# chrisquince/DESMAN

Measured on AMD Instinct MI355X. Metric: Gibbs iterations/sec (VxS updates/s) at V=10k S=64 G=8, higher is better.
Workload: dtype f64; 1 GPU; synthetic V=10000 x S=64, G=8, full Gibbs iteration, 1 chain per GPU (configs[2]); V=10000, S=64, G=8, chains=1, tau_rng=mt19937

## Files before the change

### desman_amd/_lib.py

```python
import ctypes as C
import os

import numpy as np

_HERE = os.path.dirname(os.path.abspath(__file__))
LIB_PATH = os.environ.get("DESMAN_HIP_LIB") or os.path.join(_HERE, "lib", "libdesman_hip.so")
AB_LIB_PATH = os.path.join(_HERE, "lib", "libdesman_hip_ab.so")
HEADER_PATH = os.path.join(os.path.dirname(_HERE), "include", "desman_hip.h")

DSM_OK = 0
RNG_MT19937, RNG_PHILOX = 0, 1
STATS_AGG = 2
K_NAMES = ("stats", "dirichlet", "tau", "finalize", "mt", "nmft_a", "nmft_gamma", "nmft_b", "stats2", "stats_big", "stats_pat")


class DesmanHipError(RuntimeError):
    pass


_i64p = np.ctypeslib.ndpointer(np.int64, flags="C_CONTIGUOUS")
_f64p = np.ctypeslib.ndpointer(np.float64, flags="C_CONTIGUOUS")
_u64p = np.ctypeslib.ndpointer(np.uint64, flags="C_CONTIGUOUS")
_u32p = np.ctypeslib.ndpointer(np.uint32, flags="C_CONTIGUOUS")
_i32p = np.ctypeslib.ndpointer(np.int32, flags="C_CONTIGUOUS")
_vp, _i, _d = C.c_void_p, C.c_int, C.c_double

SIGNATURES = {
    "dsm_last_error": (C.c_char_p, []),
    "dsm_device_count": (_i, []),
    "dsm_version": (C.c_char_p, []),
    "dsm_initRNG": (_i, []),
    "dsm_setRNG": (_i, [C.c_ulong]),
    "dsm_freeRNG": (_i, []),
    "dsm_sample_tau": (_i, [_i64p, _f64p, _f64p, _i64p, _i, _i, _i]),
    "c_initRNG": (None, []),
    "c_setRNG": (None, [C.c_ulong]),
    "c_freeRNG": (None, []),
    "c_sample_tau": (_i, [_i64p, _f64p, _f64p, _i64p, _i, _i, _i]),
    "dsm_getRNG_state": (_i, [_u32p]),
    "dsm_setRNG_state": (_i, [_u32p]),
    "dsm_ctx_create": (_i, [C.POINTER(_vp), _i]),
    "dsm_ctx_destroy": (_i, [_vp]),
    "dsm_ctx_sync": (_i, [_vp]),
    "dsm_ctx_set_counts": (_i, [_vp, _i64p, _i, _i]),
    "dsm_ctx_set_state": (_i, [_vp, _i64p, _f64p, _f64p, _i]),
    "dsm_ctx_get_state": (_i, [_vp, _vp, _vp, _vp]),
    "dsm_ctx_set_gamma_eta": (_i, [_vp, _vp, _vp]),
    "dsm_ctx_set_priors": (_i, [_vp, _d, _d, _d]),
    "dsm_ctx_seed": (_i, [_vp, C.c_ulong, C.c_uint64]),
    "dsm_ctx_set_tau_rng": (_i, [_vp, _i]),
    "dsm_ctx_get_mt_state": (_i, [_vp, _u32p]),
    "dsm_ctx_set_mt_state": (_i, [_vp, _u32p]),
    "dsm_mt_seed_state": (_i, [C.c_ulong, _u32p]),
    "dsm_ctx_debug_mt_fill": (_i, [_vp, C.c_size_t, _u32p]),
    "dsm_ctx_sample_tau": (_i, [_vp, C.POINTER(_i), _vp]),
    "dsm_ctx_sample_stats": (_i, [_vp, C.c_uint32, _u64p, _u64p]),
    "dsm_ctx_stats_spec": (_i, [_vp]),
    "dsm_ctx_sweep_stats": (_i, [_vp, C.POINTER(C.c_uint64), C.POINTER(C.c_uint64), _i]),
    "dsm_ctx_set_tau_screen": (_i, [_vp, _i]),
    "dsm_ctx_set_tau_neartie": (_i, [_vp, _i]),
    "dsm_ctx_set_nmft_fused": (_i, [_vp, _i]),
    "dsm_ctx_set_nmft_persist": (_i, [_vp, _i]),
    "dsm_ctx_tau_launch_info": (_i, [_vp, C.POINTER(_i), C.POINTER(_i)]),
    "dsm_ctx_debug_log2f": (_i, [_vp, _vp, _vp, C.c_size_t]),
    "dsm_debug_fdiv": (_i, [_i, _f64p, _f64p, _f64p, _i]),
    "dsm_release_device_caches": (_i, []),
    "dsm_ctx_force_stats_spec": (_i, [_vp, _i]),
    "dsm_ctx_debug_stage1": (_i, [_vp, C.c_uint32, _vp, _u64p]),
    "dsm_ctx_debug_binom": (_i, [_vp, _i, C.c_uint32, _f64p, C.c_uint64, _i, _u32p, _i]),
    "dsm_ctx_draw_gamma_eta": (_i, [_vp, C.c_uint32, _u64p, _u64p, _f64p, _f64p]),
    "dsm_ctx_loglik": (_i, [_vp, C.POINTER(_d), C.POINTER(_d)]),
    "dsm_ctx_gibbs_update": (_i, [_vp, _i]),
    "dsm_ctx_get_counters": (_i, [_vp, C.POINTER(C.c_uint64), C.POINTER(C.c_uint32)]),
    "dsm_ctx_set_counters": (_i, [_vp, C.c_uint64, C.c_uint32]),
    "dsm_ctx_get_screen_state": (_i, [_vp, _u32p]),
    "dsm_ctx_set_screen_state": (_i, [_vp, _u32p]),
    "dsm_ctx_gibbs_update_sharded": (_i, [_vp, _i, _i, _i, _vp, _vp]),
    "dsm_ctx_gibbs_update_sharded_comm": (_i, [_vp, _i, _i, _i, _vp]),
    "dsm_comm_unique_id": (_i, [_vp]),
    "dsm_comm_create": (_i, [C.POINTER(_vp), _vp, _i, _i, _i]),
    "dsm_comm_destroy": (_i, [_vp]),
    "dsm_comm_rank": (_i, [_vp]),
    "dsm_comm_world": (_i, [_vp]),
    "dsm_comm_allgather_f64": (_i, [_vp, _f64p, _f64p, C.c_size_t]),
    "dsm_comm_allreduce_f64": (_i, [_vp, _vp, C.c_size_t, _i]),
    "dsm_comm_barrier": (_i, [_vp]),
    "dsm_device_read": (_i, [_i, _vp, _vp, C.c_size_t]),
    "dsm_device_write": (_i, [_i, _vp, _vp, C.c_size_t]),
    "dsm_batch_gibbs_update": (_i, [C.POINTER(_vp), _i, _i]),
    "dsm_batch_update_tau": (_i, [C.POINTER(_vp), _i, _i, C.POINTER(_vp), C.POINTER(_vp)]),
    "dsm_batch_nmft_factorize": (_i, [C.POINTER(_vp), _i, _i, _d, _i, C.POINTER(_i), _vp]),
    "dsm_ctx_update_tau": (_i, [_vp, _i, _f64p, _f64p]),
    "dsm_ctx_get_trace": (_i, [_vp, _vp, _vp, _vp, _vp, _vp]),
    "dsm_ctx_get_star": (_i, [_vp, _vp, _vp, _vp, C.POINTER(_d), C.POINTER(_i)]),
    "dsm_ctx_get_tau_sum": (_i, [_vp, _i64p]),
    "dsm_ctx_get_tau_at": (_i, [_vp, _i, _i64p]),
    "dsm_nmft_set": (_i, [_vp, _f64p, _f64p, _i]),
    "dsm_nmft_get": (_i, [_vp, _vp, _vp]),
    "dsm_nmft_factorize": (_i, [_vp, _i, _d, _i, C.POINTER(_i), _vp]),
    "dsm_nmft_objective": (_i, [_vp, C.POINTER(_d)]),
    "dsm_nmft_get_tau": (_i, [_vp, _i64p]),
    "dsm_lrt_step": (_i, [_i, _f64p, _i32p, _i32p, _f64p, _d, _i, _i, _f64p, _f64p, _f64p]),
    "dsm_assign_tau": (_i, [_i, _i64p, _i, _i, _i, _f64p, _f64p, C.c_uint64, _vp, _vp, _vp, _vp, _vp]),
    "dsm_ctx_assign_tau": (_i, [_vp, _f64p, _f64p, _i, C.c_uint64, _vp, _vp, _vp, _vp, _vp]),
    "dsm_assign_debug_set_chunk": (_i, [_i]),
    "dsm_genes_create": (_i, [C.POINTER(_vp), _i]),
    "dsm_genes_destroy": (_i, [_vp]),
    "dsm_genes_set_data": (_i, [_vp, _vp, _i, _i, _i, _i32p, _f64p]),
    "dsm_genes_set_model": (_i, [_vp, _f64p, _f64p, _f64p, _i, _i, _f64p, _f64p, _f64p]),
    "dsm_genes_set_state": (_i, [_vp, _vp, _vp]),
    "dsm_genes_get_state": (_i, [_vp, _vp, _vp]),
    "dsm_genes_seed": (_i, [_vp, C.c_ulong, C.c_uint64]),
    "dsm_genes_set_gene_base": (_i, [_vp, _i]),
    "dsm_genes_get_mt_state": (_i, [_vp, _u32p]),
    "dsm_genes_set_mt_state": (_i, [_vp, _u32p]),
    "dsm_genes_nmft_tau": (_i, [_vp, _vp, _f64p, _i, _d, _vp]),
    "dsm_genes_sweep_all": (_i, [_vp, _vp, _i, _vp, _vp, _vp]),
    "dsm_genes_step_candidates": (_i, [_vp, _i, _i, _f64p, _vp]),
    "dsm_genes_step_choose": (_i, [_vp, _i, _i, _i]),
    "dsm_genes_update": (_i, [_vp, _i, _i, _vp, _vp, _vp, _vp]),
    "dsm_genes_loglik": (_i, [_vp, _vp]),
    "dsm_genes_get_star": (_i, [_vp, _vp, _vp]),
    "dsm_genes_set_star": (_i, [_vp, _vp, _vp]),
    "dsm_kl_assign": (_i, [_i, _f64p, _f64p, _f64p, _i, _i, _i, _i, _d, C.POINTER(_i), C.POINTER(_d)]),
    "dsm_ctx_set_timing": (_i, [_vp, _i]),
    "dsm_ctx_get_timing": (_i, [_vp, _vp, _vp]),
    "dsm_kernel_name": (C.c_char_p, [_i]),
}

EXCHANGE_FN = C.CFUNCTYPE(C.c_int, C.c_void_p, C.c_void_p, C.c_size_t, C.c_void_p, C.c_size_t)
_lib = None


def _digest(a):
    try:
        import xxhash
        return xxhash.xxh3_128_digest(memoryview(a).cast("B"))
    except ImportError:
        import hashlib
        return hashlib.blake2b(memoryview(a).cast("B"), digest_size=16).digest()


def load():
    global _lib
    if _lib is None:
        if not os.path.exists(LIB_PATH):
            raise DesmanHipError(
                "libdesman_hip.so not built (%s); run `python -c 'import __graft_entry__ as g; g.build()'` "
                "or `make -C desman_amd/csrc`.  There is no CPU fallback." % LIB_PATH)
        try:
            lib = C.CDLL(LIB_PATH)
# ... 181 lines not shown
    def restore(self, ck):
        self.set_state(np.ascontiguousarray(ck["tau"], dtype=np.int64), np.ascontiguousarray(ck["gamma"], dtype=np.float64),
                       np.ascontiguousarray(ck["eta"], dtype=np.float64))
        mt = np.asarray(ck["mt_state"], dtype=np.uint32)
        if mt.size == 625:
            self.set_mt_state(np.ascontiguousarray(mt))
        check(self.lib.dsm_ctx_set_counters(self._h, int(ck["ctr_seed"]), int(ck["iter_ctr"])))
        self.set_screen_state(ck["screen"] if "screen" in ck else np.zeros(2, dtype=np.uint32))

    def set_mt_state(self, st):
        check(self.lib.dsm_ctx_set_mt_state(self._h, np.ascontiguousarray(st, dtype=np.uint32)))

    def debug_mt_fill(self, n):
        out = np.empty(int(n), dtype=np.uint32)
        check(self.lib.dsm_ctx_debug_mt_fill(self._h, int(n), out))
        return out

    def set_tau_rng(self, mode):
        check(self.lib.dsm_ctx_set_tau_rng(self._h, int(mode)))

    def assign_tau(self, gamma, eta, seed=None):
        gamma, eta = _assign_model(gamma, eta, self.S)
        G = gamma.shape[1]
        out = _assign_out(self.V, G, seed)
        check(self.lib.dsm_ctx_assign_tau(self._h, gamma, eta, G, int(seed or 0) & 0xFFFFFFFFFFFFFFFF, _ptr(out["map_state"]),
                                          _ptr(out["conf"]), _ptr(out["logz"]), _ptr(out["marg"]), _ptr(out.get("draw_state"))))
        return out

    def sample_tau(self, want_logp=False):
        n = _i(0)
        logp = np.empty((self.V, self.G, 4)) if want_logp else None
        check(self.lib.dsm_ctx_sample_tau(self._h, C.byref(n), _ptr(logp)))
        return (n.value, logp) if want_logp else n.value

    def sample_stats(self, it):
        mu = np.zeros((self.S, self.G), dtype=np.uint64)
        E = np.zeros((4, 4), dtype=np.uint64)
        check(self.lib.dsm_ctx_sample_stats(self._h, int(it), mu, E))
        return mu, E

    def debug_log2f(self, x):
        x = np.ascontiguousarray(x, dtype=np.float32)
        out = np.empty_like(x)
        check(self.lib.dsm_ctx_debug_log2f(self._h, x.ctypes.data, out.ctypes.data, x.size))
        return out

    def set_tau_neartie(self, mode=-1):
        check(self.lib.dsm_ctx_set_tau_neartie(self._h, int(mode)))

    def set_tau_screen(self, on):
        check(self.lib.dsm_ctx_set_tau_screen(self._h, 1 if on else 0))

    def tau_launch_info(self):
        a, b = _i(0), _i(0)
        check(self.lib.dsm_ctx_tau_launch_info(self._h, C.byref(a), C.byref(b)))
        return a.value, b.value

    def set_nmft_persist(self, mode=-1):
        check(self.lib.dsm_ctx_set_nmft_persist(self._h, int(mode)))

    def set_nmft_fused(self, mode=-1):
        check(self.lib.dsm_ctx_set_nmft_fused(self._h, int(mode)))

    def sweep_stats(self, reset=False):
        a, b = C.c_uint64(0), C.c_uint64(0)
        check(self.lib.dsm_ctx_sweep_stats(self._h, C.byref(a), C.byref(b), 1 if reset else 0))
        return a.value, b.value

    def stats_spec(self):
        r = self.lib.dsm_ctx_stats_spec(self._h)
        if r < 0:
            check(r)
        return r

    def force_stats_spec(self, spec=0):
        check(self.lib.dsm_ctx_force_stats_spec(self._h, int(spec)))

    def debug_stage1(self, it):
        nt = np.zeros((self.S, 1 << self.G), dtype=np.uint32)
        E = np.zeros((4, 4), dtype=np.uint64)
        check(self.lib.dsm_ctx_debug_stage1(self._h, int(it), nt.ctypes.data, E))
        return nt, E

    def debug_binom(self, kind, n, w, seed, nsamp, spec=STATS_AGG):
        w4 = np.zeros(4)
        w4[:len(w)] = w
        out = np.zeros((nsamp, 4) if kind == 2 else nsamp, dtype=np.uint32)
        check(self.lib.dsm_ctx_debug_binom(self._h, int(kind), int(n), w4, int(seed), int(nsamp), out.reshape(-1), int(spec)))
        return out

    def draw_gamma_eta(self, it, sum_mu, esum):
        g = np.empty((self.S, self.G)); e = np.empty((4, 4))
        check(self.lib.dsm_ctx_draw_gamma_eta(self._h, int(it), np.ascontiguousarray(sum_mu, dtype=np.uint64),
                                              np.ascontiguousarray(esum, dtype=np.uint64), g, e))
        return g, e

    def loglik(self):
        ll, lp = _d(0), _d(0)
        check(self.lib.dsm_ctx_loglik(self._h, C.byref(ll), C.byref(lp)))
        return ll.value, lp.value

    def gibbs_update(self, n_iter):
        check(self.lib.dsm_ctx_gibbs_update(self._h, int(n_iter)))
        self.n_trace = int(n_iter)

    def gibbs_update_sharded(self, n_iter, v_offset, v_total, exchange):
        err = []

        def cb(user, tab, n_tab, vec, n_vec):
            try:
                exchange(tab or 0, int(n_tab), vec, int(n_vec))
                return 0
            except BaseException as e:
                err.append(e)
                return 1
        fn = EXCHANGE_FN(cb)
        rc = self.lib.dsm_ctx_gibbs_update_sharded(self._h, int(n_iter), int(v_offset), int(v_total), C.cast(fn, _vp), None)
        if err:
            raise err[0]
        check(rc)
        self.n_trace = int(n_iter)

    def gibbs_update_sharded_comm(self, n_iter, v_offset, v_total, comm):
        check(self.lib.dsm_ctx_gibbs_update_sharded_comm(self._h, int(n_iter), int(v_offset), int(v_total), comm._h))
        self.n_trace = int(n_iter)

    @staticmethod
    def batch_gibbs_update(ctxs, n_iter):
        ctxs = list(ctxs)
        arr = (_vp * len(ctxs))(*[c._h.value for c in ctxs])
        check(load().dsm_batch_gibbs_update(arr, len(ctxs), int(n_iter)))
        for c in ctxs:
            c.n_trace = int(n_iter)

    def update_tau(self, gamma_store, eta_store):
        g = np.ascontiguousarray(gamma_store, dtype=np.float64)
        e = np.ascontiguousarray(eta_store, dtype=np.float64)
        check(self.lib.dsm_ctx_update_tau(self._h, g.shape[0], g, e))
        self.n_trace = g.shape[0]

    def get_trace(self):
        n = self.n_trace
        ll = np.empty(n); lp = np.empty(n); nch = np.empty(n, dtype=np.int32)
        g = np.empty((n, self.S, self.G)); e = np.empty((n, 4, 4))
        check(self.lib.dsm_ctx_get_trace(self._h, _ptr(ll), _ptr(lp), _ptr(nch), _ptr(g), _ptr(e)))
        return dict(ll=ll, lp=lp, nchange=nch, gamma=g, eta=e)

    def get_star(self):
        tau = np.empty((self.V, self.G, 4), dtype=np.int64)
        g = np.empty((self.S, self.G)); e = np.empty((4, 4))
        lp, it = _d(0), _i(0)
        check(self.lib.dsm_ctx_get_star(self._h, _ptr(tau), _ptr(g), _ptr(e), C.byref(lp), C.byref(it)))
        return dict(tau=tau, gamma=g, eta=e, lp=lp.value, it=it.value)

    def get_tau_sum(self):
        out = np.empty((self.V, self.G, 4), dtype=np.int64)
        check(self.lib.dsm_ctx_get_tau_sum(self._h, out))
        return out

    def get_tau_at(self, it):
        out = np.empty((self.V, self.G, 4), dtype=np.int64)
        check(self.lib.dsm_ctx_get_tau_at(self._h, int(it), out))
        return out

    def nmft_set(self, tau, gamma):
        tau = np.ascontiguousarray(tau, dtype=np.float64)
# ... 186 lines not shown
```

### desman_amd/csrc/api.hip

```cpp
#include <math.h>
#include <stdarg.h>
#include <stdio.h>
#include <string.h>

#include <algorithm>
#include <mutex>
#include <numeric>
#include <thread>

#include "dsm_host.h"
#include "log_table.h"

static thread_local char g_err[512] = "";

void dsm_set_error(const char *fmt, ...)
{
    va_list ap;
    va_start(ap, fmt);
    vsnprintf(g_err, sizeof g_err, fmt, ap);
    va_end(ap);
}

extern "C" const char *dsm_last_error(void) { return g_err; }
extern "C" const char *dsm_version(void) { return "desman_hip 0.1 (gfx950)"; }
// ... 113 lines not shown
    static const std::vector<uint32_t> ident = [] { std::vector<uint32_t> v((size_t)2 * DSM_MAX_GRID); for (size_t i = 0; i < v.size(); ++i) v[i] = (uint32_t)(i % DSM_MAX_GRID); return v; }();
    c->blk_order_n[0] = c->blk_order_n[1] = 0;
    if (!c->blk_order) return DSM_OK;
    HIP_TRY(hipMemcpyAsync(c->blk_order, ident.data(), ident.size() * sizeof(uint32_t), hipMemcpyHostToDevice, c->stream));
    return DSM_OK;
}

extern "C" int dsm_ctx_create(dsm_ctx **out, int device)
{
    if (!out) return DSM_ERR_ARG;
    *out = nullptr;
    int n = dsm_device_count();
    if (n <= 0) { dsm_set_error("no HIP device visible"); return DSM_ERR_NODEVICE; }
    if (device < 0 || device >= n) { dsm_set_error("device %d out of range (0..%d)", device, n - 1); return DSM_ERR_ARG; }
    HIP_TRY(hipSetDevice(device));
    hipDeviceProp_t prop;
    HIP_TRY(hipGetDeviceProperties(&prop, device));
    if (strncmp(prop.gcnArchName, "gfx950", 6) != 0) {
        dsm_set_error("device %d is %s; this library is built for gfx950 only", device, prop.gcnArchName);
        return DSM_ERR_NODEVICE;
    }
    dsm_ctx *c = new dsm_ctx();
    c->device = device;
    HIP_TRY(hipStreamCreateWithFlags(&c->stream, hipStreamNonBlocking));
    if (getenv("DESMAN_HIP_ONE_STREAM")) c->stream_rng = c->stream;
    else {
        int lo = 0, hi = 0;
        HIP_TRY(hipDeviceGetStreamPriorityRange(&lo, &hi));
        HIP_TRY(hipStreamCreateWithPriority(&c->stream_rng, hipStreamNonBlocking, hi));
    }
    for (int i = 0; i < 2; ++i) {
        HIP_TRY(hipEventCreateWithFlags(&c->ev_u_ready[i], hipEventDisableTiming));
        HIP_TRY(hipEventCreateWithFlags(&c->ev_u_free[i], hipEventDisableTiming));
    }
    TRY(dev_alloc(&c->mt_state, 625));
    TRY(dev_alloc(&c->ll_partial, 2 * DSM_MAX_GRID));
    TRY(dev_alloc(&c->nchange, 2));
    TRY(dev_alloc(&c->sweep_stats, 2));
    HIP_TRY(hipMemsetAsync(c->sweep_stats, 0, 2 * sizeof(unsigned long long), c->stream));
    TRY(dev_alloc(&c->step_cnt, (size_t)2 * 2 * DSM_MAX_GRID));
    HIP_TRY(hipMemsetAsync(c->step_cnt, 0, (size_t)2 * 2 * DSM_MAX_GRID * sizeof(uint32_t), c->stream));
    TRY(dev_alloc(&c->blk_order, (size_t)2 * DSM_MAX_GRID));
    TRY(reset_blk_order(c));
    TRY(dev_alloc(&c->screen_ctl, 4));
    HIP_TRY(hipMemsetAsync(c->screen_ctl, 0, 4 * sizeof(uint32_t), c->stream));
    TRY(dev_alloc(&c->prior, 2 * (DSM_MAX_S + 4)));
    TRY(dev_alloc(&c->scalars, 8));
    TRY(dev_alloc(&c->star, 2));
    TRY(dev_alloc(&c->eta, 16));
    TRY(dev_alloc(&c->eta_new, 16));
    TRY(dev_alloc(&c->eta_star, 16));
    TRY(dev_alloc(&c->esum, 16 + 16 * DSM_ESUM_PARTS));
    TRY(dev_alloc(&c->log_tab, 2 * DSM_LOG_TAB_N + DSM_EXP_TAB_N));
    HIP_TRY(hipMemcpyAsync(c->log_tab, dsm_log_table_host, sizeof dsm_log_table_host, hipMemcpyHostToDevice, c->stream));
    HIP_TRY(hipMemcpyAsync(c->log_tab + 2 * DSM_LOG_TAB_N, dsm_exp_table_host, sizeof dsm_exp_table_host, hipMemcpyHostToDevice, c->stream));
    HIP_TRY(hipMemsetAsync(c->nchange, 0, 2 * sizeof(int), c->stream));
    TRY(esum_reset(c));
    HIP_TRY(hipStreamSynchronize(c->stream));
    *out = c;
    return DSM_OK;
}

static void free_traces(dsm_ctx *c)
{
    dev_free(&c->tau_trace); dev_free(&c->ll_trace); dev_free(&c->lp_trace); dev_free(&c->nchange_trace);
    dev_free(&c->gamma_trace); dev_free(&c->eta_trace); dev_free(&c->gamma_in); dev_free(&c->eta_in);
    c->in_cap = 0;
    c->n_trace = 0;
    c->trace_cap = 0;
}

extern "C" int dsm_ctx_destroy(dsm_ctx *c)
{
    if (!c) return DSM_OK;
    (void)hipSetDevice(c->device);
    (void)hipStreamSynchronize(c->stream);
    collect_spans(c);
    for (auto e : c->free_events) (void)hipEventDestroy(e);
    free_traces(c);
    dev_free(&c->cnt_vs); dev_free(&c->items); dev_free(&c->nitems); dev_free(&c->tau);
    dev_free(&c->pat_rep); dev_free(&c->pat_x); dev_free(&c->pat_list); c->pat_rep_len = c->pat_x_len = 0;
    if (c->h_rare) { (void)hipHostFree(c->h_rare); c->h_rare = nullptr; }
    dev_free(&c->s2_scratch);
    dev_free(&c->blk_tab); stats_release_ntab(c); dev_free(&c->big_list); dev_free(&c->big_count);
    dev_free(&c->gamma); dev_free(&c->eta);
    dev_free(&c->eta_new); dev_free(&c->sum_mu); dev_free(&c->esum); dev_free(&c->mt_state); dev_free(&c->mt_jstates); dev_free(&c->u_raw);
    dev_free(&c->ll_partial); dev_free(&c->nchange); dev_free(&c->sweep_stats); dev_free(&c->step_cnt); dev_free(&c->blk_order); dev_free(&c->screen_ctl); dev_free(&c->prior); dev_free(&c->prior_all); dev_free(&c->scalars); dev_free(&c->star);
    dev_free(&c->gamma_star); dev_free(&c->eta_star); dev_free(&c->log_tab); dev_free(&c->shard_vec); dev_free(&c->np_part); if (c->np_bar) { (void)hipFree(c->np_bar); c->np_bar = nullptr; } dev_free(&c->F); dev_free(&c->ntau); dev_free(&c->ntau2); dev_free(&c->ngam); dev_free(&c->ngam_raw);
    dev_free(&c->npart); dev_free(&c->nstat); dev_free(&c->ngam2); dev_free(&c->ngam_raw2);
    for (int i = 0; i < 2; ++i) { (void)hipEventDestroy(c->ev_u_ready[i]); (void)hipEventDestroy(c->ev_u_free[i]); }
    if (c->stream_rng != c->stream) (void)hipStreamDestroy(c->stream_rng);
    (void)hipStreamDestroy(c->stream);
    delete c;
    return DSM_OK;
}

extern "C" int dsm_ctx_sync(dsm_ctx *c)
{
    if (!c) return DSM_ERR_ARG;
    BIND(c);
    HIP_TRY(hipStreamSynchronize(c->stream));
    HIP_TRY(hipStreamSynchronize(c->stream_rng));
    return DSM_OK;
}

extern "C" int dsm_ctx_set_counts(dsm_ctx *c, const int64_t *variants, int V, int S)
{
    if (!c || !variants || V < 1 || S < 1) { dsm_set_error("set_counts: bad arguments"); return DSM_ERR_ARG; }
    if (S > DSM_MAX_S) { dsm_set_error("S=%d exceeds DSM_MAX_S=%d", S, DSM_MAX_S); return DSM_ERR_UNSUPPORTED; }
    if ((int64_t)V * S >= ((int64_t)1 << 32)) { dsm_set_error("V*S must be below 2^32"); return DSM_ERR_UNSUPPORTED; }
    BIND(c);
    HIP_TRY(hipStreamSynchronize(c->stream));
    HIP_TRY(hipStreamSynchronize(c->stream_rng));
    const size_t n = (size_t)V * S;
    c->V = V; c->S = S;
    c->have_state = false;
    c->G = 0;
    TRY(dev_alloc(&c->cnt_vs, n * 4));
    TRY(dev_alloc(&c->nitems, (size_t)S));
    TRY(dev_alloc(&c->tau, (size_t)V));
    dev_free(&c->F); dev_free(&c->ntau); dev_free(&c->ntau2); dev_free(&c->ngam); dev_free(&c->ngam_raw); c->nG = 0;
    free_traces(c);
    Scratch<int64_t> d_in; Scratch<int> d_flag; Scratch<double> d_part; Scratch<unsigned long long> d_depth;
    const int nblk = (int)((n + 255) / 256 < 1024 ? (n + 255) / 256 : 1024);
    TRY(d_in.alloc(n * 4));
    TRY(d_flag.alloc(1));
    TRY(d_part.alloc((size_t)nblk));
    TRY(d_depth.alloc((size_t)S));
    HIP_TRY(hipMemcpyAsync(d_in, variants, n * 4 * sizeof(int64_t), hipMemcpyHostToDevice, c->stream));
    HIP_TRY(hipMemsetAsync(d_flag, 0, sizeof(int), c->stream));
    HIP_TRY(hipMemsetAsync(d_depth, 0, (size_t)S * sizeof(unsigned long long), c->stream));
    TRY(k_convert_counts(c, d_in, d_flag, d_part, nblk, d_depth));
    std::vector<double> part(nblk);
    std::vector<unsigned long long> dep((size_t)S);
    int flag = 0;
    HIP_TRY(hipMemcpyAsync(part.data(), d_part, nblk * sizeof(double), hipMemcpyDeviceToHost, c->stream));
    HIP_TRY(hipMemcpyAsync(dep.data(), d_depth, (size_t)S * sizeof(unsigned long long), hipMemcpyDeviceToHost, c->stream));
    HIP_TRY(hipMemcpyAsync(&flag, d_flag, sizeof(int), hipMemcpyDeviceToHost, c->stream));
    HIP_TRY(hipStreamSynchronize(c->stream));
    c->items_built = false;
    c->max_items = 0;
    c->blk_gmax = 0;
    c->stats_grid = 0;
    dev_free(&c->pat_x); c->pat_x_len = 0;
    TRY(reset_blk_order(c));
    HIP_TRY(hipMemsetAsync(c->screen_ctl, 0, 4 * sizeof(uint32_t), c->stream));
    dev_free(&c->items);
    c->depth.assign((size_t)S, 0);
    c->max_depth = 0;
    for (int s = 0; s < S; ++s) { c->depth[s] = (int64_t)dep[s]; c->max_depth = std::max<uint64_t>(c->max_depth, dep[s]); }
    if (flag) {
        dev_free(&c->cnt_vs); dev_free(&c->items);
        dsm_set_error("set_counts: negative count or depth above 2^31-1");
        return DSM_ERR_ARG;
    }
    double s = 0.0;
    for (double p : part) s += p;
    c->ll_const = s;
    return DSM_OK;
}

int build_stats_items(dsm_ctx *c)
{
    const int V = c->V, S = c->S;
    std::vector<int32_t> cnt((size_t)V * S * 4);
    HIP_TRY(hipMemcpyAsync(cnt.data(), c->cnt_vs, cnt.size() * sizeof(int32_t), hipMemcpyDeviceToHost, c->stream));
    HIP_TRY(hipStreamSynchronize(c->stream));
    const int64_t cells = (int64_t)V * S;
    const int CH = cells <= 65536 ? 64 : cells <= 262144 ? 128 : 0;
    c->chunked = CH != 0;
    std::vector<int32_t> nit(S);
    std::vector<std::vector<std::pair<int32_t, int32_t>>> lst((size_t)S);
    std::vector<int32_t> top(S, 0);
    for (int s = 0; s < S; ++s) lst[s].reserve((size_t)V * 2);
    for (int v = 0; v < V; ++v) {
        const int32_t *row = cnt.data() + (size_t)v * S * 4;
        for (int s = 0; s < S; ++s)
            for (int b = 0; b < 4; ++b) {
                const int64_t x = row[s * 4 + b];
                if (x <= 0) continue;
                if (!CH) {
                    lst[s].emplace_back((int32_t)x, v * 4 + b);
                    if (x > top[s]) top[s] = (int32_t)x;
                } else {
                    for (int64_t j = 0; j * CH < x; ++j) {
                        const int32_t nrd = (int32_t)(x - j * CH < CH ? x - j * CH : CH);
                        lst[s].emplace_back(nrd | (int32_t)(j << 12), v * 4 + b);
                        if (nrd > top[s]) top[s] = nrd;
                    }
                }
            }
    }
    int max_items = 0;
    for (int s = 0; s < S; ++s) max_items = std::max(max_items, (int)lst[s].size());
    c->item_stride = max_items > 0 ? max_items : 1;
    std::vector<int32_t> items((size_t)S * c->item_stride * 2, 0);
    TRY(dev_alloc(&c->items, items.size()));
    std::vector<int32_t> first;
    const int32_t rd_mask = CH ? 0xfff : 0x7fffffff;
    for (int s = 0; s < S; ++s) {
        const auto &l = lst[s];
        nit[s] = (int32_t)l.size();
        int32_t *dst = items.data() + (size_t)s * c->item_stride * 2;
        if (top[s] <= (1 << 20)) {
            first.assign((size_t)top[s] + 2, 0);
            for (const auto &e : l) first[e.first & rd_mask]++;
            int32_t run = 0;
            for (int32_t cval = top[s]; cval >= 1; --cval) { const int32_t h = first[cval]; first[cval] = run; run += h; }
            for (const auto &e : l) { const int32_t k = first[e.first & rd_mask]++; dst[2 * k] = e.second; dst[2 * k + 1] = e.first; }
        } else {
            std::vector<std::pair<int32_t, int32_t>> t(l);
            std::stable_sort(t.begin(), t.end(), [](const std::pair<int32_t, int32_t> &p, const std::pair<int32_t, int32_t> &q) { return p.first > q.first; });
            for (size_t k = 0; k < t.size(); ++k) { dst[2 * k] = t[k].second; dst[2 * k + 1] = t[k].first; }
        }
    }
    c->max_items = max_items;
    c->nitems_h = nit;
    c->blk_gmax = 0;
    HIP_TRY(hipMemcpyAsync(c->items, items.data(), items.size() * sizeof(int32_t), hipMemcpyHostToDevice, c->stream));
    HIP_TRY(hipMemcpyAsync(c->nitems, nit.data(), (size_t)S * sizeof(int32_t), hipMemcpyHostToDevice, c->stream));
    HIP_TRY(hipStreamSynchronize(c->stream));
    c->items_built = true;
    return DSM_OK;
}

static int ensure_state_buffers(dsm_ctx *c, int G)
{
    if (G < 1 || G > DSM_MAX_G) { dsm_set_error("G=%d outside 1..%d", G, DSM_MAX_G); return DSM_ERR_UNSUPPORTED; }
    if (G != c->G || !c->gamma) {
        c->G = G;
        const size_t sg = (size_t)c->S * G;
        TRY(dev_alloc(&c->gamma, sg));
        TRY(dev_alloc(&c->gamma_star, sg));
        TRY(dev_alloc(&c->sum_mu, sg));
        HIP_TRY(hipMemsetAsync(c->sum_mu, 0, sg * sizeof(unsigned long long), c->stream));
        c->stats_grid = 0;
        c->u_cap = (size_t)c->V * G;
        c->u_chunk_words = c->u_cap * std::max<size_t>(1, std::min<size_t>(DSM_U_CHUNK, ((size_t)16 << 20) / std::max<size_t>(1, c->u_cap)));
        TRY(dev_alloc(&c->u_raw, 2 * c->u_chunk_words));
        free_traces(c);
    }
    return DSM_OK;
}

extern "C" int dsm_ctx_set_state(dsm_ctx *c, const int64_t *tau, const double *gamma, const double *eta, int G)
{
    TRY(need(c, true, false));
    if (!tau || !gamma || !eta) { dsm_set_error("set_state: null pointer"); return DSM_ERR_ARG; }
    BIND(c);
    HIP_TRY(hipStreamSynchronize(c->stream));
    TRY(ensure_state_buffers(c, G));
    const size_t nt = (size_t)c->V * G * 4;
    Scratch<int64_t> d_t;
    TRY(d_t.alloc(nt));
    HIP_TRY(hipMemcpyAsync(d_t, tau, nt * sizeof(int64_t), hipMemcpyHostToDevice, c->stream));
    TRY(k_pack_tau(c, d_t, c->tau, c->V, G));
    HIP_TRY(hipMemcpyAsync(c->gamma, gamma, (size_t)c->S * G * sizeof(double), hipMemcpyHostToDevice, c->stream));
    c->tau_rare_n = tau_rare_from_host(gamma, c->S, G);
    HIP_TRY(hipMemcpyAsync(c->eta, eta, 16 * sizeof(double), hipMemcpyHostToDevice, c->stream));
    HIP_TRY(hipStreamSynchronize(c->stream));
    c->have_state = true;
    return DSM_OK;
}

extern "C" int dsm_ctx_set_gamma_eta(dsm_ctx *c, const double *gamma, const double *eta)
{
    TRY(need(c, true, true));
    BIND(c);
    if (gamma) HIP_TRY(hipMemcpyAsync(c->gamma, gamma, (size_t)c->S * c->G * sizeof(double), hipMemcpyHostToDevice, c->stream));
    if (gamma) c->tau_rare_n = tau_rare_from_host(gamma, c->S, c->G);
    if (eta) HIP_TRY(hipMemcpyAsync(c->eta, eta, 16 * sizeof(double), hipMemcpyHostToDevice, c->stream));
    HIP_TRY(hipStreamSynchronize(c->stream));
    return DSM_OK;
}

static int fetch_tau(dsm_ctx *c, const uint64_t *d_packed, int64_t *host_onehot)
{
    const size_t nt = (size_t)c->V * c->G * 4;
    Scratch<int64_t> d_t;
    TRY(d_t.alloc(nt));
    TRY(k_unpack_tau(c, d_packed, d_t, c->V, c->G));
    HIP_TRY(hipMemcpyAsync(host_onehot, d_t, nt * sizeof(int64_t), hipMemcpyDeviceToHost, c->stream));
    HIP_TRY(hipStreamSynchronize(c->stream));
    return DSM_OK;
}

extern "C" int dsm_ctx_get_state(dsm_ctx *c, int64_t *tau, double *gamma, double *eta)
{
    TRY(need(c, true, true));
    BIND(c);
    if (tau) TRY(fetch_tau(c, c->tau, tau));
    if (gamma) HIP_TRY(hipMemcpyAsync(gamma, c->gamma, (size_t)c->S * c->G * sizeof(double), hipMemcpyDeviceToHost, c->stream));
    if (eta) HIP_TRY(hipMemcpyAsync(eta, c->eta, 16 * sizeof(double), hipMemcpyDeviceToHost, c->stream));
    HIP_TRY(hipStreamSynchronize(c->stream));
    return DSM_OK;
}

extern "C" int dsm_ctx_set_priors(dsm_ctx *c, double alpha, double delta, double epsilon)
{
    if (!c || !(alpha > 0) || !(delta > 0) || !(epsilon >= 0)) { dsm_set_error("set_priors: bad value"); return DSM_ERR_ARG; }
    c->alpha = alpha; c->delta = delta; c->epsilon = epsilon;
    return DSM_OK;
}

static void mt_seed_host(uint32_t *st, unsigned long seed)
{
    if (seed == 0) seed = 4357;
    st[0] = (uint32_t)(seed & 0xffffffffUL);
    for (int i = 1; i < 624; ++i) st[i] = 1812433253u * (st[i - 1] ^ (st[i - 1] >> 30)) + (uint32_t)i;
    st[624] = 624;
}

static int seed_mt(dsm_ctx *c, unsigned long seed)
{
    uint32_t st[625];
    mt_seed_host(st, seed);
    HIP_TRY(hipStreamSynchronize(c->stream_rng));
    HIP_TRY(hipMemcpyAsync(c->mt_state, st, sizeof st, hipMemcpyHostToDevice, c->stream));
    HIP_TRY(hipStreamSynchronize(c->stream));
// ... 143 lines not shown
        for (int slot = 0; slot < 2; ++slot)
            if (len[slot] && it == first[slot] + len[slot] - 1) HIP_TRY(hipEventRecord(c->ev_u_free[slot], c->stream));
        return DSM_OK;
    }
};

extern "C" int dsm_ctx_sample_tau(dsm_ctx *c, int *nchange, double *logp_out)
{
    TRY(need(c, true, true));
    BIND(c);
    Scratch<double> d_logp;
    const size_t nl = (size_t)c->V * c->G * 4;
    if (logp_out) TRY(d_logp.alloc(nl));
    const uint32_t *u = nullptr;
    SweepWords words(c, 1);
    HIP_TRY(hipMemsetAsync(c->nchange, 0, sizeof(int), c->stream));
    TRY(words.acquire(0, &u));
    TRY(k_tau_sweep(c, 1, c->gamma, c->eta, c->eta, nullptr, d_logp, c->iter_ctr++, nullptr, u));
    TRY(words.release(0));
    int n = 0;
    HIP_TRY(hipMemcpyAsync(&n, c->nchange, sizeof(int), hipMemcpyDeviceToHost, c->stream));
    if (logp_out) HIP_TRY(hipMemcpyAsync(logp_out, d_logp, nl * sizeof(double), hipMemcpyDeviceToHost, c->stream));
    HIP_TRY(hipMemsetAsync(c->nchange, 0, sizeof(int), c->stream));
    HIP_TRY(hipStreamSynchronize(c->stream));
    if (nchange) *nchange = n;
    return DSM_OK;
}

extern "C" int dsm_ctx_sample_stats(dsm_ctx *c, uint32_t iter, uint64_t *sum_mu, uint64_t *esum)
{
    TRY(need(c, true, true));
    BIND(c);
    const size_t sg = (size_t)c->S * c->G;
    HIP_TRY(hipMemsetAsync(c->sum_mu, 0, sg * sizeof(unsigned long long), c->stream));
    TRY(stats_ensure_ntab(c));
    TRY(esum_reset(c));
    TRY(k_stats(c, iter));
    TRY(k_esum_fold(c));
    if (sum_mu) HIP_TRY(hipMemcpyAsync(sum_mu, c->sum_mu, sg * sizeof(uint64_t), hipMemcpyDeviceToHost, c->stream));
    if (esum) HIP_TRY(hipMemcpyAsync(esum, c->esum, 16 * sizeof(uint64_t), hipMemcpyDeviceToHost, c->stream));
    HIP_TRY(hipMemsetAsync(c->sum_mu, 0, sg * sizeof(unsigned long long), c->stream));
    TRY(esum_reset(c));
    HIP_TRY(hipStreamSynchronize(c->stream));
    return DSM_OK;
}

extern "C" int dsm_ctx_stats_spec(dsm_ctx *c)
{
    if (!c || c->G < 1) { dsm_set_error("stats_spec: no chain state"); return DSM_ERR_STATE; }
    return stats_spec(c);
}

extern "C" int dsm_ctx_force_stats_spec(dsm_ctx *c, int spec)
{
    if (!c || spec < 0 || spec > 4) { dsm_set_error("force_stats_spec: 0 (rule), 1, 2, 3 or 4"); return DSM_ERR_ARG; }
    c->force_stats_spec = spec;
    return DSM_OK;
}

extern "C" int dsm_ctx_debug_stage1(dsm_ctx *c, uint32_t iter, uint32_t *ntab, uint64_t *esum)
{
    TRY(need(c, true, true));
    if (stats_spec(c) < 2) { dsm_set_error("debug_stage1: the aggregated specification does not apply to this shape (force it with dsm_ctx_force_stats_spec)"); return DSM_ERR_UNSUPPORTED; }
    BIND(c);
    TRY(esum_reset(c));
    TRY(k_stats_stage1(c, iter));
    TRY(k_esum_fold(c));
    const size_t NH = (size_t)1 << c->G, S = (size_t)c->S;
    const size_t ld = (size_t)c->ntab_ld;
    std::vector<uint32_t> t((size_t)c->ntab_rep * NH * ld);
    HIP_TRY(hipMemcpyAsync(t.data(), c->ntab, t.size() * sizeof(uint32_t), hipMemcpyDeviceToHost, c->stream));
    if (esum) HIP_TRY(hipMemcpyAsync(esum, c->esum, 16 * sizeof(uint64_t), hipMemcpyDeviceToHost, c->stream));
    HIP_TRY(hipMemsetAsync(c->ntab, 0, t.size() * sizeof(uint32_t), c->stream));
    TRY(esum_reset(c));
    HIP_TRY(hipMemsetAsync(c->big_count, 0, DSM_BIG_NT * DSM_BIG_NL * DSM_BIG_STRIDE * sizeof(uint32_t), c->stream));
    HIP_TRY(hipStreamSynchronize(c->stream));
    if (ntab)
        for (size_t h = 0; h < NH; ++h)
            for (size_t s = 0; s < S; ++s) {
                uint32_t v = 0;
                for (int r = 0; r < c->ntab_rep; ++r) v += t[((size_t)r * NH + ((h * DSM_NTAB_HMUL + (s >> 4) * DSM_NTAB_SWZ) & (NH - 1))) * ld + s];
                ntab[s * NH + h] = v;
            }
    return DSM_OK;
}

extern "C" int dsm_ctx_debug_binom(dsm_ctx *c, int kind, uint32_t n, const double *w4, uint64_t seed, int nsamp, uint32_t *out, int spec)
{
    if (!c || !w4 || !out || nsamp < 1 || kind < 0 || kind > 2 || spec < 2 || spec > 3) { dsm_set_error("debug_binom: bad arguments"); return DSM_ERR_ARG; }
    BIND(c);
    const size_t len = (size_t)nsamp * (kind == 2 ? 4 : 1);
    Scratch<uint32_t> d;
    TRY(d.alloc(len));
    TRY(k_binom_test(c, kind, n, w4, seed, nsamp, d, spec));
    HIP_TRY(hipMemcpyAsync(out, d, len * sizeof(uint32_t), hipMemcpyDeviceToHost, c->stream));
    HIP_TRY(hipStreamSynchronize(c->stream));
    return DSM_OK;
}

extern "C" int dsm_ctx_draw_gamma_eta(dsm_ctx *c, uint32_t iter, const uint64_t *sum_mu, const uint64_t *esum,
                                      double *gamma_out, double *eta_out)
{
    TRY(need(c, true, true));
    if (!sum_mu || !esum) { dsm_set_error("draw_gamma_eta: null sums"); return DSM_ERR_ARG; }
    BIND(c);
    const size_t sg = (size_t)c->S * c->G;
    Scratch<double> d_g, d_e;
    TRY(d_g.alloc(sg));
    TRY(d_e.alloc(16));
    HIP_TRY(hipMemcpyAsync(c->sum_mu, sum_mu, sg * sizeof(uint64_t), hipMemcpyHostToDevice, c->stream));
    HIP_TRY(hipMemcpyAsync(c->esum, esum, 16 * sizeof(uint64_t), hipMemcpyHostToDevice, c->stream));
    TRY(k_dirichlet(c, iter, d_g, nullptr, d_e, nullptr, c->prior, -1, 0, nullptr));
    if (gamma_out) HIP_TRY(hipMemcpyAsync(gamma_out, d_g, sg * sizeof(double), hipMemcpyDeviceToHost, c->stream));
    if (eta_out) HIP_TRY(hipMemcpyAsync(eta_out, d_e, 16 * sizeof(double), hipMemcpyDeviceToHost, c->stream));
    HIP_TRY(hipStreamSynchronize(c->stream));
    return DSM_OK;
}

static int eval_state(dsm_ctx *c, const double *gamma, const double *eta, uint64_t *trace_slot, int star_mode)
{
    int nb = 0;
    TRY(k_prior(c, gamma, eta, c->prior));
    TRY(k_tau_sweep(c, 2, gamma, eta, eta, trace_slot, nullptr, 0, &nb, nullptr));
    return k_finalize(c, nb, -1, star_mode, c->prior, gamma, eta);
}

extern "C" int dsm_ctx_loglik(dsm_ctx *c, double *ll, double *lp)
{
    TRY(need(c, true, true));
    BIND(c);
    double sc[2];
    TRY(eval_state(c, c->gamma, c->eta, nullptr, 2));
    HIP_TRY(hipMemcpyAsync(sc, c->scalars, sizeof sc, hipMemcpyDeviceToHost, c->stream));
    HIP_TRY(hipStreamSynchronize(c->stream));
    if (ll) *ll = sc[0];
    if (lp) *lp = sc[1];
    return DSM_OK;
}

static int alloc_traces(dsm_ctx *c, int n)
{
    const size_t sg = (size_t)c->S * c->G;
    if (n > c->trace_cap || !c->tau_trace) {
        free_traces(c);
        const int want = n;
        if (n < 512 && (size_t)513 * c->V * sizeof(uint64_t) <= ((size_t)1 << 30)) n = 512;
        TRY(dev_alloc(&c->tau_trace, (size_t)(n + 1) * c->V));
        TRY(dev_alloc(&c->ll_trace, (size_t)n));
        TRY(dev_alloc(&c->lp_trace, (size_t)n));
        TRY(dev_alloc(&c->nchange_trace, (size_t)n));
        TRY(dev_alloc(&c->gamma_trace, (size_t)n * sg));
        TRY(dev_alloc(&c->eta_trace, (size_t)n * 16));
        c->trace_cap = n;
        n = want;
    }
    c->n_trace = n;
    return DSM_OK;
}

thread_local BatchCtl g_batch;

struct Chains {
    dsm_ctx *const *c;
    int K;
    bool batched;
    struct Home { hipStream_t stream, stream_rng; bool timing; int nmft_fused; };
    std::vector<Home> home;
    dsm_ctx *lead() const { return c[0]; }
    ~Chains()
    {
        if (home.empty()) return;
        (void)hipStreamSynchronize(lead()->stream);
        (void)hipStreamSynchronize(lead()->stream_rng);
        for (size_t k = 0; k < home.size(); ++k) {
            c[k]->stream = home[k].stream; c[k]->stream_rng = home[k].stream_rng; c[k]->timing = home[k].timing; c[k]->nmft_fused = home[k].nmft_fused;
        }
    }
    template <class Fits> int open(bool state, bool nmft, Fits fits)
    {
        if (!c || K < 1 || K > DSM_MAX_BATCH) { dsm_set_error("batch of %d chains (1..%d)", K, DSM_MAX_BATCH); return DSM_ERR_ARG; }
        for (int k = 0; k < K; ++k) {
            TRY(need(c[k], true, state));
            const dsm_ctx *a = c[0], *b = c[k];
            if (b->device != a->device || b->V != a->V || b->S != a->S) { dsm_set_error("batch: chain %d differs from chain 0 in device or shape", k); return DSM_ERR_ARG; }
            TRY(fits(a, b, k));
            for (int j = 0; j < k; ++j) if (c[j] == b) { dsm_set_error("batch: chain %d listed twice", k); return DSM_ERR_ARG; }
        }
        BIND(lead());
        for (int k = 0; batched && k < K; ++k) {
            HIP_TRY(hipStreamSynchronize(c[k]->stream));
            HIP_TRY(hipStreamSynchronize(c[k]->stream_rng));
            home.push_back(Home{c[k]->stream, c[k]->stream_rng, c[k]->timing, c[k]->nmft_fused});
            c[k]->stream = lead()->stream; c[k]->stream_rng = lead()->stream_rng; c[k]->timing = false;
            if (nmft) c[k]->nmft_fused = home[0].nmft_fused;
        }
        return DSM_OK;
    }
    template <class F> int each(F f) const
    {
        for (int k = 0; k < K; ++k) TRY(f(c[k], k));
        return DSM_OK;
    }
    template <class F> int launch(F f) const
    {
        int r = DSM_OK;
        for (int k = 0; k < K && r == DSM_OK; ++k) {
            if (batched) g_batch = BatchCtl{K, k};
            r = f(c[k], k);
        }
        g_batch = BatchCtl{};
        return r;
    }
};

static int same_G_and_rng(const dsm_ctx *a, const dsm_ctx *b, int k)
{
    if (b->G != a->G || b->tau_rng != a->tau_rng) { dsm_set_error("batch: chain %d differs from chain 0 in shape or tau RNG", k); return DSM_ERR_ARG; }
    return DSM_OK;
}

static double *prior_slot(dsm_ctx *c, int it) { return c->prior + (it & 1) * (DSM_MAX_S + 4); }

static int gibbs_update(dsm_ctx *const *ctxs, int K, bool batched, int n_iter)
{
    if (n_iter < 0) { dsm_set_error("n_iter < 0"); return DSM_ERR_ARG; }
    Chains ch{ctxs, K, batched};
    TRY(ch.open(true, false, [](const dsm_ctx *a, const dsm_ctx *b, int k) -> int {
        TRY(same_G_and_rng(a, b, k));
        if (stats_spec(b) == stats_spec(a)) return DSM_OK;
        dsm_set_error("batch: chain %d runs mu/E specification %d, chain 0 specification %d (different tables or different dsm_ctx_force_stats_spec)", k, stats_spec(b), stats_spec(a));
        return DSM_ERR_ARG;
    }));
    dsm_ctx *const lead = ch.lead();
    const int spec = stats_spec(lead);
    const bool agg = spec >= 2;
    const bool fuse_s2 = agg && lead->G < 10;
    const size_t sg = (size_t)lead->S * lead->G;
    std::vector<SweepWords> words;
    words.reserve(K);
    std::vector<int> nb_prev(K, 0);
    std::vector<uint32_t> ic(K);
    std::vector<const uint32_t *> u(K, nullptr);
    TRY(ch.each([&](dsm_ctx *c, int) -> int {
        TRY(alloc_traces(c, n_iter));
        HIP_TRY(hipMemsetAsync(c->nchange, 0, sizeof(int), c->stream));
        TRY(eval_state(c, c->gamma, c->eta, c->tau_trace, 1));
        TRY(stats_ensure_ntab(c));
        if (!batched) TRY(k_tau_neartie_hint(c));
        words.emplace_back(c, n_iter);
        return DSM_OK;
    }));
    TRY(ch.launch([&](dsm_ctx *, int k) { return words[k].prefetch(); }));
    for (int it = 0; it < n_iter; ++it) {
        if (!batched && it && (it & 63) == 0 && lead->tau_neartie_mode == -1) { TRY(k_tau_rare_count(lead, true)); TRY(k_tau_neartie_hint(lead)); }
        TRY(ch.launch([&](dsm_ctx *c, int k) { ic[k] = c->iter_ctr++; return agg ? k_stats_stage1(c, ic[k]) : k_stats_v1(c, ic[k]); }));
        if (agg && !fuse_s2) TRY(ch.launch([&](dsm_ctx *c, int k) { return k_stats_stage2(c, ic[k]); }));
        TRY(ch.launch([&](dsm_ctx *c, int k) {
            return k_dirichlet(c, ic[k], c->gamma, c->gamma_trace + (size_t)it * sg, c->eta_new, c->eta_trace + (size_t)it * 16,
                               prior_slot(c, it), it - 1, nb_prev[k], prior_slot(c, it - 1), fuse_s2 ? 1 : 0);
        }));
        TRY(ch.launch([&](dsm_ctx *, int k) { return words[k].acquire(it, &u[k]); }));
        TRY(ch.launch([&](dsm_ctx *c, int k) {
            return k_tau_sweep(c, 3, c->gamma, c->eta, c->eta_new, c->tau_trace + (size_t)(it + 1) * c->V, nullptr, ic[k], &nb_prev[k], u[k]);
        }));
        TRY(ch.each([&](dsm_ctx *c, int k) -> int {
            TRY(words[k].release(it));
            std::swap(c->eta, c->eta_new);
            return DSM_OK;
        }));
    }
    const bool want_rare = !batched && n_iter > 0 && lead->tau_neartie_mode == -1;
    if (want_rare && !lead->h_rare) HIP_TRY(hipHostMalloc((void **)&lead->h_rare, sizeof(int), hipHostMallocDefault));
    if (n_iter > 0)
        TRY(ch.each([&](dsm_ctx *c, int k) {
            return k_finalize(c, nb_prev[k], n_iter - 1, 0, prior_slot(c, n_iter - 1), c->gamma_trace + (size_t)(n_iter - 1) * sg,
                              c->eta_trace + (size_t)(n_iter - 1) * 16, 0, want_rare ? c->h_rare : nullptr);
        }));
    HIP_TRY(hipStreamSynchronize(lead->stream));
    if (want_rare) lead->tau_rare_n = *lead->h_rare;
    return DSM_OK;
}

extern "C" int dsm_ctx_gibbs_update(dsm_ctx *c, int n_iter) { return gibbs_update(&c, 1, false, n_iter); }

extern "C" int dsm_batch_gibbs_update(dsm_ctx *const *ctxs, int K, int n_iter) { return gibbs_update(ctxs, K, true, n_iter); }

struct dsm_comm;
int comm_enqueue_exchange(dsm_comm *m, uint32_t *tab, size_t n_tab, double *vec, size_t n_vec, hipStream_t stream);
int comm_device(const dsm_comm *m);

static int gibbs_update_sharded(dsm_ctx *c, int n_iter, int v_offset, int v_total, dsm_exchange_fn exchange, void *user, dsm_comm *comm)
{
    TRY(need(c, true, true));
    c->tau_neartie_on = false;
    if (n_iter < 0 || (!exchange && !comm) || v_offset < 0 || v_total < v_offset + c->V) { dsm_set_error("gibbs_update_sharded: bad arguments"); return DSM_ERR_ARG; }
    if (comm && comm_device(comm) != c->device) { dsm_set_error("gibbs_update_sharded: the communicator lives on device %d, the context on %d", comm_device(comm), c->device); return DSM_ERR_ARG; }
    if (c->tau_rng != DSM_RNG_PHILOX) { dsm_set_error("gibbs_update_sharded: needs counter-based tau uniforms (DSM_RNG_PHILOX)"); return DSM_ERR_STATE; }
    BIND(c);
    const int keep_force = c->force_stats_spec;
    if (c->force_stats_spec < 2) c->force_stats_spec = DSM_STATS_AGG;
    struct Guard { dsm_ctx *c; int f; ~Guard() { c->shard_on = false; c->force_stats_spec = f; } } guard{c, keep_force};
    if (stats_spec(c) < 2) { dsm_set_error("gibbs_update_sharded: the aggregated mu/E pass does not apply to this shape (G <= 16)"); return DSM_ERR_UNSUPPORTED; }
    if (!c->shard_vec) TRY(dev_alloc(&c->shard_vec, (size_t)18));
    c->shard_on = true; c->shard_voff = v_offset; c->shard_vtot = v_total;
    TRY(alloc_traces(c, n_iter));
    const size_t sg = (size_t)c->S * c->G;
    HIP_TRY(hipMemsetAsync(c->nchange, 0, sizeof(int), c->stream));
    TRY(esum_reset(c));
    auto swap_vec = [&](uint32_t *tab, size_t n_tab) -> int {
        if (comm) return comm_enqueue_exchange(comm, tab, n_tab, c->shard_vec, (size_t)18, c->stream);
        HIP_TRY(hipStreamSynchronize(c->stream));
        if (exchange(user, tab, n_tab, c->shard_vec, (size_t)18) != 0) { dsm_set_error("gibbs_update_sharded: the exchange callback failed"); return DSM_ERR_STATE; }
        return DSM_OK;
    };
    {
        int nb = 0;
        TRY(k_prior(c, c->gamma, c->eta, c->prior));
        TRY(k_tau_sweep(c, 2, c->gamma, c->eta, c->eta, c->tau_trace, nullptr, 0, &nb, nullptr));
        TRY(k_shard_pack(c, nb));
        TRY(swap_vec(nullptr, 0));
        TRY(k_finalize(c, nb, -1, 1, c->prior, c->gamma, c->eta));
        TRY(esum_reset(c));
    }
    TRY(stats_ensure_ntab(c));
    double *const P[2] = {c->prior, c->prior + (DSM_MAX_S + 4)};
    int nb_prev = 0;
    for (int it = 0; it < n_iter; ++it) {
        const uint32_t ic = c->iter_ctr++;
        const bool fuse_s2 = c->G < 10;
        TRY(k_stats_stage1(c, ic));
        TRY(k_shard_pack(c, nb_prev));
        TRY(swap_vec(c->ntab, c->ntab_len));
        TRY(k_shard_unpack(c));
        if (!fuse_s2) TRY(k_stats_stage2(c, ic));
        TRY(k_dirichlet(c, ic, c->gamma, c->gamma_trace + (size_t)it * sg, c->eta_new, c->eta_trace + (size_t)it * 16,
                        P[it & 1], it - 1, nb_prev, P[(it - 1) & 1], fuse_s2 ? 1 : 0));
        TRY(k_tau_sweep(c, 3, c->gamma, c->eta, c->eta_new, c->tau_trace + (size_t)(it + 1) * c->V, nullptr, ic, &nb_prev, nullptr));
        std::swap(c->eta, c->eta_new);
    }
    if (n_iter > 0) {
        TRY(k_shard_pack(c, nb_prev));
        TRY(swap_vec(nullptr, 0));
        TRY(k_finalize(c, nb_prev, n_iter - 1, 0, P[(n_iter - 1) & 1], c->gamma_trace + (size_t)(n_iter - 1) * sg,
                       c->eta_trace + (size_t)(n_iter - 1) * 16));
        TRY(esum_reset(c));
    }
    HIP_TRY(hipStreamSynchronize(c->stream));
    return DSM_OK;
}

extern "C" int dsm_ctx_gibbs_update_sharded(dsm_ctx *c, int n_iter, int v_offset, int v_total, dsm_exchange_fn exchange, void *user)
{
    if (!exchange) { dsm_set_error("gibbs_update_sharded: no exchange callback"); return DSM_ERR_ARG; }
    return gibbs_update_sharded(c, n_iter, v_offset, v_total, exchange, user, nullptr);
}

extern "C" int dsm_ctx_gibbs_update_sharded_comm(dsm_ctx *c, int n_iter, int v_offset, int v_total, dsm_comm *comm)
{
    if (!comm) { dsm_set_error("gibbs_update_sharded_comm: no communicator"); return DSM_ERR_ARG; }
    return gibbs_update_sharded(c, n_iter, v_offset, v_total, nullptr, nullptr, comm);
}

// ... 35 lines not shown
    if (n_iter < 1 || !gamma_stores || !eta_stores) { dsm_set_error("update_tau: bad arguments"); return DSM_ERR_ARG; }
    Chains ch{ctxs, K, batched};
    TRY(ch.open(true, false, [&](const dsm_ctx *a, const dsm_ctx *b, int k) {
        if (!gamma_stores[k] || !eta_stores[k]) { dsm_set_error("update_tau: bad arguments"); return DSM_ERR_ARG; }
        return same_G_and_rng(a, b, k);
    }));
    const size_t sg = (size_t)ch.lead()->S * ch.lead()->G;
    std::vector<SweepWords> words;
    words.reserve(K);
    TRY(ch.each([&](dsm_ctx *c, int) -> int { TRY(alloc_traces(c, n_iter)); words.emplace_back(c, n_iter); return DSM_OK; }));
    TRY(ch.launch([&](dsm_ctx *, int k) { return words[k].prefetch(); }));
    TRY(ch.each([&](dsm_ctx *c, int k) { return tau_inputs(c, n_iter, gamma_stores[k], eta_stores[k]); }));
    std::vector<int> nb_prev(K, 0);
    std::vector<const uint32_t *> u(K, nullptr);
    for (int it = 0; it < n_iter; ++it) {
        TRY(ch.launch([&](dsm_ctx *, int k) { return words[k].acquire(it, &u[k]); }));
        TRY(ch.launch([&](dsm_ctx *c, int k) -> int {
            const uint32_t ic = c->iter_ctr++;
            const double *g = c->gamma_in + (size_t)it * sg, *e = c->eta_in + (size_t)it * 16;
            TauFinalRider rider;
            if (it > 0) {
                rider.nblocks = nb_prev[k]; rider.it = it - 1; rider.prior = c->prior_all + (size_t)(it - 1) * (c->S + 4);
                rider.gamma_src = c->gamma_in + (size_t)(it - 1) * sg; rider.eta_src = c->eta_in + (size_t)(it - 1) * 16;
            }
            return k_tau_sweep(c, 3, g, e, e, c->tau_trace + (size_t)(it + 1) * c->V, nullptr, ic, &nb_prev[k], u[k], it & 1,
                               it > 0 ? &rider : nullptr);
        }));
        TRY(ch.each([&](dsm_ctx *, int k) { return words[k].release(it); }));
    }
    TRY(ch.each([&](dsm_ctx *c, int k) {
        return k_finalize(c, nb_prev[k], n_iter - 1, 0, c->prior_all + (size_t)(n_iter - 1) * (c->S + 4),
                          c->gamma_in + (size_t)(n_iter - 1) * sg, c->eta_in + (size_t)(n_iter - 1) * 16, (n_iter - 1) & 1);
    }));
    HIP_TRY(hipStreamSynchronize(ch.lead()->stream));
    return DSM_OK;
}

extern "C" int dsm_ctx_update_tau(dsm_ctx *c, int n_iter, const double *gamma_store, const double *eta_store) { return update_tau(&c, 1, false, n_iter, &gamma_store, &eta_store); }

extern "C" int dsm_batch_update_tau(dsm_ctx *const *ctxs, int K, int n_iter, const double *const *gamma_stores, const double *const *eta_stores)
{
    return update_tau(ctxs, K, true, n_iter, gamma_stores, eta_stores);
}

extern "C" int dsm_release_device_caches(void)
{
    mt_jump_release();
    return DSM_OK;
}

extern "C" int dsm_ctx_debug_log2f(dsm_ctx *c, const float *in, float *out, size_t n)
{
    if (!c || !in || !out) { dsm_set_error("debug_log2f: bad arguments"); return DSM_ERR_ARG; }
    if (n == 0) return DSM_OK;
    BIND(c);
    Scratch<float> d_in, d_out;
    TRY(d_in.alloc(n)); TRY(d_out.alloc(n));
    HIP_TRY(hipMemcpyAsync(d_in, in, n * sizeof(float), hipMemcpyHostToDevice, c->stream));
    TRY(k_log2f_test(c, d_in, d_out, n));
    HIP_TRY(hipMemcpyAsync(out, d_out, n * sizeof(float), hipMemcpyDeviceToHost, c->stream));
    HIP_TRY(hipStreamSynchronize(c->stream));
    return DSM_OK;
}

extern "C" int dsm_ctx_tau_launch_info(dsm_ctx *c, int *launched, int *resident)
{
    TRY(need(c, true, true));
    if (!launched || !resident) { dsm_set_error("tau_launch_info: null argument"); return DSM_ERR_ARG; }
    BIND(c);
    return tau_launch_info(c, launched, resident);
}

extern "C" int dsm_ctx_set_nmft_persist(dsm_ctx *c, int mode)
{
    if (!c || mode < -1 || mode > 1) { dsm_set_error("set_nmft_persist: mode -1, 0 or 1"); return DSM_ERR_ARG; }
    c->nmft_persist = mode;
    return DSM_OK;
}

extern "C" int dsm_ctx_set_nmft_fused(dsm_ctx *c, int mode)
{
    if (!c || mode < -1 || mode > 3 || mode == 2) { dsm_set_error("set_nmft_fused: mode -1, 0, 1 or 3"); return DSM_ERR_ARG; }
    c->nmft_fused = mode;
    return DSM_OK;
}

extern "C" int dsm_ctx_set_tau_neartie(dsm_ctx *c, int mode)
{
    if (!c || mode < -1 || mode > 1) { dsm_set_error("set_tau_neartie: -1 (by the abundances), 0 or 1"); return DSM_ERR_ARG; }
    c->tau_neartie_mode = mode;
    return DSM_OK;
}

extern "C" int dsm_ctx_set_tau_screen(dsm_ctx *c, int on)
{
    if (!c) { dsm_set_error("set_tau_screen: null context"); return DSM_ERR_ARG; }
    c->tau_screen = on != 0;
    return DSM_OK;
}

extern "C" int dsm_ctx_sweep_stats(dsm_ctx *c, uint64_t *steps, uint64_t *exact_steps, int mode)
{
    if (!c || mode < 0 || mode > 1) { dsm_set_error("sweep_stats: bad arguments"); return DSM_ERR_ARG; }
    BIND(c);
    unsigned long long h[2] = {0, 0};
    HIP_TRY(hipMemcpyAsync(h, c->sweep_stats, sizeof h, hipMemcpyDeviceToHost, c->stream));
    if (mode == 1) HIP_TRY(hipMemsetAsync(c->sweep_stats, 0, sizeof h, c->stream));
    HIP_TRY(hipStreamSynchronize(c->stream));
    if (steps) *steps = h[0];
    if (exact_steps) *exact_steps = h[1];
    return DSM_OK;
}

extern "C" int dsm_ctx_get_trace(dsm_ctx *c, double *ll, double *lp, int32_t *nchange, double *gamma_store, double *eta_store)
{
    TRY(need(c, true, true));
    BIND(c);
    const size_t n = (size_t)c->n_trace, sg = (size_t)c->S * c->G;
    if (n == 0) return DSM_OK;
    if (ll) HIP_TRY(hipMemcpyAsync(ll, c->ll_trace, n * sizeof(double), hipMemcpyDeviceToHost, c->stream));
    if (lp) HIP_TRY(hipMemcpyAsync(lp, c->lp_trace, n * sizeof(double), hipMemcpyDeviceToHost, c->stream));
    if (nchange) HIP_TRY(hipMemcpyAsync(nchange, c->nchange_trace, n * sizeof(int), hipMemcpyDeviceToHost, c->stream));
    if (gamma_store) HIP_TRY(hipMemcpyAsync(gamma_store, c->gamma_trace, n * sg * sizeof(double), hipMemcpyDeviceToHost, c->stream));
    if (eta_store) HIP_TRY(hipMemcpyAsync(eta_store, c->eta_trace, n * 16 * sizeof(double), hipMemcpyDeviceToHost, c->stream));
    HIP_TRY(hipStreamSynchronize(c->stream));
    return DSM_OK;
}

extern "C" int dsm_ctx_get_star(dsm_ctx *c, int64_t *tau_star, double *gamma_star, double *eta_star, double *lp_star, int *iter_star)
{
    TRY(need(c, true, true));
    if (!c->tau_trace) { dsm_set_error("get_star: no update has run"); return DSM_ERR_STATE; }
    BIND(c);
    double st[2];
    HIP_TRY(hipMemcpyAsync(st, c->star, sizeof st, hipMemcpyDeviceToHost, c->stream));
    HIP_TRY(hipStreamSynchronize(c->stream));
    const int slot = (int)st[1];
    if (tau_star) TRY(fetch_tau(c, c->tau_trace + (size_t)slot * c->V, tau_star));
    if (gamma_star) HIP_TRY(hipMemcpyAsync(gamma_star, c->gamma_star, (size_t)c->S * c->G * sizeof(double), hipMemcpyDeviceToHost, c->stream));
    if (eta_star) HIP_TRY(hipMemcpyAsync(eta_star, c->eta_star, 16 * sizeof(double), hipMemcpyDeviceToHost, c->stream));
    HIP_TRY(hipStreamSynchronize(c->stream));
    if (lp_star) *lp_star = st[0];
    if (iter_star) *iter_star = slot > 0 ? slot - 1 : 0;
    return DSM_OK;
}

extern "C" int dsm_ctx_get_tau_sum(dsm_ctx *c, int64_t *tau_sum)
{
    TRY(need(c, true, true));
    if (!c->tau_trace || !tau_sum) { dsm_set_error("get_tau_sum: no update has run"); return DSM_ERR_STATE; }
    BIND(c);
    const size_t nt = (size_t)c->V * c->G * 4;
    Scratch<int64_t> d;
    TRY(d.alloc(nt));
    TRY(k_tau_sum(c, c->tau_trace, c->n_trace, d));
    HIP_TRY(hipMemcpyAsync(tau_sum, d, nt * sizeof(int64_t), hipMemcpyDeviceToHost, c->stream));
    HIP_TRY(hipStreamSynchronize(c->stream));
    return DSM_OK;
}

extern "C" int dsm_ctx_get_tau_at(dsm_ctx *c, int it, int64_t *tau)
{
    TRY(need(c, true, true));
    if (!c->tau_trace || !tau || it < -1 || it >= c->n_trace) { dsm_set_error("get_tau_at: bad iteration"); return DSM_ERR_ARG; }
    BIND(c);
    return fetch_tau(c, c->tau_trace + (size_t)(it + 1) * c->V, tau);
// ... 335 lines not shown
```

### desman_amd/csrc/dsm_host.h

```cpp
#pragma once
#include <hip/hip_runtime.h>
#include <stdint.h>
#include <string>
#include <vector>

#include "../../include/desman_hip.h"

#define DSM_MAX_GRID 4096
#define DSM_ESUM_PARTS 64
#define DSM_BIG_NL 64
#define DSM_BIG_STRIDE 16
#define DSM_BIG_NT 3
#define DSM_U_CHUNK 8

#define DSM_STATS_AGG 2
#define DSM_MAX_BATCH 8

void dsm_set_error(const char *fmt, ...);

#ifdef DSM_AB_SWITCHES
#define DSM_AB_ENV(name) getenv(name)
#else
#define DSM_AB_ENV(name) ((const char *)nullptr)
#endif

struct BatchCtl { int K = 0, k = 0; };
extern thread_local BatchCtl g_batch;
template <class P> struct BatchArgs { P p[DSM_MAX_BATCH]; };
#define LAUNCH_OR_COLLECT(PT, P, NORMAL, BATCHED)                                          \
    do {                                                                                    \
        if (g_batch.K == 0) { NORMAL; }                                                     \
        else {                                                                              \
            static thread_local BatchArgs<PT> acc;                                          \
            acc.p[g_batch.k] = (P);                                                         \
            if (g_batch.k == g_batch.K - 1) { const int K = g_batch.K; (void)K; BATCHED; }  \
        }                                                                                   \
    } while (0)

#define HIP_TRY(expr)                                                                       \
    do {                                                                                    \
        hipError_t _e = (expr);                                                             \
        if (_e != hipSuccess) {                                                             \
            dsm_set_error("%s failed: %s (%s:%d)", #expr, hipGetErrorString(_e), __FILE__, \
                          __LINE__);                                                        \
            return DSM_ERR_HIP;                                                             \
        }                                                                                   \
    } while (0)

struct TimedSpan { int k; hipEvent_t e0, e1; };

struct dsm_ctx {
    int device = 0;
    hipStream_t stream = nullptr;
    hipStream_t stream_rng = nullptr;
    hipEvent_t ev_u_ready[2] = {nullptr, nullptr}, ev_u_free[2] = {nullptr, nullptr};
    int V = 0, S = 0, G = 0;
    int32_t *cnt_vs = nullptr;
    int32_t *items = nullptr;
    int32_t *nitems = nullptr;
    int max_items = 0;
    bool items_built = false;
    uint64_t max_depth = 0;
    int force_stats_spec = 0;
    uint32_t *ntab = nullptr;
    size_t ntab_len = 0;
    unsigned long long *pat_rep = nullptr;
    uint32_t *pat_x = nullptr;
    uint32_t *pat_list = nullptr;
    size_t pat_rep_len = 0, pat_x_len = 0;
    uint32_t pat_gen = 0;
    uint32_t *s2_scratch = nullptr;
    uint32_t *ntab_raw = nullptr;
    int ntab_ld = 0;
    int ntab_rep = 1;
    unsigned long long *big_list = nullptr;
    uint32_t *big_count = nullptr;
    size_t big_cap = 0;
    int stats_grid = 0;
    int stats_grid_key = -1;
    int item_stride = 1;
    bool chunked = false;
    int32_t *blk_tab = nullptr;
    int blk_n = 0, blk_gmax = 0;
    std::vector<int64_t> depth;
    std::vector<int32_t> nitems_h;
    double ll_const = 0.0;
    uint64_t *tau = nullptr;
    double *gamma = nullptr;
    double *eta = nullptr;
    double *eta_new = nullptr;
    bool have_state = false;
    double alpha = 0.1, delta = 0.1, epsilon = 1e-6;
    unsigned long long *sum_mu = nullptr;
    unsigned long long *esum = nullptr;
    uint32_t *mt_state = nullptr;
    uint32_t *mt_jstates = nullptr;
    bool mt_seeded = false;
    uint32_t *u_raw = nullptr;
    size_t u_cap = 0;
    size_t u_chunk_words = 0;
    bool mt_attr_set = false;
    uint64_t ctr_seed = 0x243F6A8885A308D3ull;
    uint32_t iter_ctr = 0;
    int tau_rng = DSM_RNG_MT19937;
    double *ll_partial = nullptr;
    int *nchange = nullptr;
    unsigned long long *sweep_stats = nullptr;
    uint32_t *blk_order = nullptr;
    int tau_resident = 0, tau_resident_key = -1;
    int blk_order_n[2] = {0, 0};
    uint32_t *step_cnt = nullptr;
    uint32_t *screen_ctl = nullptr;
    bool tau_screen = true;
    int tau_neartie_mode = -1;
    bool tau_neartie_on = false;
    int tau_rare_n = 0;
    int *h_rare = nullptr;
    double *prior_all = nullptr;
    double *prior = nullptr;
    double *scalars = nullptr;
    double *log_tab = nullptr;
    int n_trace = 0, trace_cap = 0;
    uint64_t *tau_trace = nullptr;
    double *ll_trace = nullptr, *lp_trace = nullptr;
    int *nchange_trace = nullptr;
    double *gamma_trace = nullptr;
    double *eta_trace = nullptr;
    double *gamma_in = nullptr, *eta_in = nullptr;
    int in_cap = 0;
    double *star = nullptr;
    double *gamma_star = nullptr;
    double *eta_star = nullptr;
    bool shard_on = false;
    int shard_voff = 0, shard_vtot = 0;
    double *shard_vec = nullptr;
    double *F = nullptr;
    double *ntau = nullptr;
    double *ntau2 = nullptr;
    double *ngam = nullptr;
    double *ngam_raw = nullptr;
    int npart_cols = 0;
    double *npart = nullptr;
    double *nstat = nullptr;
    double *ndiv_trace = nullptr;
    int nG = 0;
    int nmft_blocks = 0;
    int nmft_persist = -1;
    double *np_part = nullptr;
    size_t np_cap = 0;
    unsigned *np_bar = nullptr;
    int nmft_fix_gamma = 0;
    int nmft_fused = -1;
    double *ngam2 = nullptr, *ngam_raw2 = nullptr;
    int nmft_gstep = 0, nmft_gstep_parity = 0, nmft_gstep_max_iter = 0;
    double nmft_gstep_min_change = 0.0;
    bool timing = false;
    std::vector<TimedSpan> spans;
    std::vector<hipEvent_t> free_events;
    double k_ms[DSM_K_COUNT] = {0};
    int64_t k_launches[DSM_K_COUNT] = {0};
};

struct KTimer {
    dsm_ctx *c; int k; hipStream_t st; hipEvent_t e0 = nullptr, e1 = nullptr;
    KTimer(dsm_ctx *ctx, int kid, hipStream_t stream = nullptr);
    ~KTimer();
};

int k_convert_counts(dsm_ctx *c, const int64_t *d_in, int *d_flag, double *d_partial, int nblk, unsigned long long *d_depth);
int k_pack_tau(dsm_ctx *c, const int64_t *d_onehot, uint64_t *d_packed, int V, int G);
int k_unpack_tau(dsm_ctx *c, const uint64_t *d_packed, int64_t *d_onehot, int V, int G);
int k_tau_sum(dsm_ctx *c, const uint64_t *trace, int n, int64_t *d_sum);
int k_mt_fill(dsm_ctx *c, uint32_t *out, size_t n, hipStream_t stream);
int k_stats_v1(dsm_ctx *c, uint32_t iter);
int k_log2f_test(dsm_ctx *c, const float *d_in, float *d_out, size_t n);
int build_stats_items(dsm_ctx *c);

#define DSM_NTAB_HMUL 0x9E3779B1u
#define DSM_NTAB_SWZ 17u
int stats_ensure_ntab(dsm_ctx *c);
void stats_release_ntab(dsm_ctx *c);
void mt_jump_release();
int stats_ntab_rep(const dsm_ctx *c);
int stats_spec(const dsm_ctx *c);
static inline int stats_draw_version(int spec) { return spec == 4 ? 2 : spec; }
int k_tau_neartie_hint(dsm_ctx *c);
int k_tau_rare_count(dsm_ctx *c, bool wait);
int tau_rare_from_host(const double *gamma, int S, int G);
int k_stats(dsm_ctx *c, uint32_t iter);
int k_stats_stage1(dsm_ctx *c, uint32_t iter);
int k_stats_stage2(dsm_ctx *c, uint32_t iter);
int k_binom_test(dsm_ctx *c, int kind, uint32_t n, const double *w, uint64_t seed, int nsamp, uint32_t *d_out, int spec);
int k_esum_fold(dsm_ctx *c);
int k_dirichlet(dsm_ctx *c, uint32_t iter, double *gamma_out, double *gamma_trace, double *eta_out, double *eta_trace,
                double *prior_out, int fin_it, int fin_nblocks, const double *fin_prior, int do_s2 = 0);
int k_prior(dsm_ctx *c, const double *gamma, const double *eta, double *prior_out);
int k_prior_batch(dsm_ctx *c, const double *gamma, const double *eta, int n, double *prior_out);
struct TauFinalRider { int nblocks, it; const double *prior, *gamma_src, *eta_src; };
int k_tau_sweep(dsm_ctx *c, int mode, const double *gamma, const double *eta_sweep,
                const double *eta_ll, uint64_t *trace_slot, double *d_logp, uint32_t iter, int *nblocks,
                const uint32_t *u_raw, int slot = 0, const TauFinalRider *rider = nullptr);
int tau_launch_info(dsm_ctx *c, int *launched, int *resident);
int k_shard_pack(dsm_ctx *c, int nblocks);
int k_shard_unpack(dsm_ctx *c);
int k_finalize(dsm_ctx *c, int nblocks, int it, int star_mode, const double *prior, const double *gamma_src,
               const double *eta_src, int slot = 0, int *rare_out = nullptr);

int k_nmft_freq(dsm_ctx *c);
int k_nmft_clamp(dsm_ctx *c);
int k_nmft_pass_a(dsm_ctx *c);
int k_nmft_gamma(dsm_ctx *c, int max_iter, double min_change, int fix_gamma, int adjust, int parity);
int k_nmft_reduce(dsm_ctx *c);
bool nmft_gstep_applies(const dsm_ctx *c, int fix_gamma);
int k_nmft_pass_b(dsm_ctx *c, int adjust);
int k_nmft_get_tau(dsm_ctx *c, uint64_t *d_packed);
int nmft_grid(dsm_ctx *c);
bool nmft_use_wave(const dsm_ctx *c);
bool nmft_use_mfma(const dsm_ctx *c);
bool nmft_use_wide(const dsm_ctx *c);
int nmft_wide_grid(const dsm_ctx *c);
int nmft_mfma_grid(const dsm_ctx *c, bool fix = false);
int k_nmft_wave(dsm_ctx *c, int adjust, int do_update);
int k_nmft_persist(dsm_ctx *c, int max_iter, double min_change, int fix_gamma, int adjust, int *used);
```

### desman_amd/csrc/kernels_gibbs.hip

```cpp
#include <string.h>

#include <mutex>

#include "dsm_device.h"
#include "dsm_host.h"
#include "dsm_stage2.h"
#include "log_table.h"

__global__ __launch_bounds__(256) void convert_counts_kernel(const int64_t *__restrict__ in,
                                                             int32_t *__restrict__ cnt_vs, int V, int S,
                                                             int *flag, double *partial,
                                                             unsigned long long *__restrict__ depth)
{
    __shared__ double red[256];
    __shared__ unsigned long long dep[DSM_MAX_S];
    for (int i = threadIdx.x; i < S; i += 256) dep[i] = 0ull;
    __syncthreads();
    const size_t n = (size_t)V * S;
    double acc = 0.0;
    for (size_t i = (size_t)blockIdx.x * 256 + threadIdx.x; i < n; i += (size_t)gridDim.x * 256) {
        int4 c;
        int64_t x[4];
        int64_t tot = 0;
        bool bad = false;
#pragma unroll
        for (int b = 0; b < 4; ++b) {
            x[b] = in[i * 4 + b];
            bad |= (x[b] < 0) | (x[b] > 2147483647ll);
            tot += x[b];
        }
        bad |= tot > 2147483647ll;
        if (bad) atomicOr(flag, 1);
        else if (tot) atomicAdd(&dep[i % (size_t)S], (unsigned long long)tot);
        c.x = (int)x[0]; c.y = (int)x[1]; c.z = (int)x[2]; c.w = (int)x[3];
        reinterpret_cast<int4 *>(cnt_vs)[i] = c;
        double t = lgamma((double)tot + 1.0);
#pragma unroll
        for (int b = 0; b < 4; ++b) t -= lgamma((double)x[b] + 1.0);
        acc += t;
    }
    red[threadIdx.x] = acc;
    __syncthreads();
    for (int o = 128; o >= 1; o >>= 1) {
        if ((int)threadIdx.x < o) red[threadIdx.x] += red[threadIdx.x + o];
        __syncthreads();
    }
    if (threadIdx.x == 0) partial[blockIdx.x] = red[0];
    for (int i = threadIdx.x; i < S; i += 256) if (dep[i]) atomicAdd(&depth[i], dep[i]);
}

__global__ void pack_tau_kernel(const int64_t *__restrict__ onehot, uint64_t *__restrict__ packed, int V, int G)
{
    const int v = blockIdx.x * blockDim.x + threadIdx.x;
    if (v >= V) return;
    uint64_t t = 0;
    for (int g = 0; g < G; ++g) {
        const int64_t *p = onehot + ((size_t)v * G + g) * 4;
        int idx = 0;
        for (int b = 3; b >= 0; --b) if (p[b] == 1) idx = b;
        t |= (uint64_t)idx << (2 * g);
    }
    packed[v] = t;
}

__global__ void unpack_tau_kernel(const uint64_t *__restrict__ packed, int64_t *__restrict__ onehot, int V, int G)
{
    const size_t i = (size_t)blockIdx.x * blockDim.x + threadIdx.x;
    if (i >= (size_t)V * G) return;
    const int v = (int)(i / G), g = (int)(i % G);
    const int idx = (int)((packed[v] >> (2 * g)) & 3);
    int64_t *p = onehot + i * 4;
#pragma unroll
    for (int b = 0; b < 4; ++b) p[b] = (b == idx) ? 1 : 0;
}

__global__ void tau_sum_kernel(const uint64_t *__restrict__ trace, int n, int V, int G, int64_t *__restrict__ out)
{
    const size_t i = (size_t)blockIdx.x * blockDim.x + threadIdx.x;
    if (i >= (size_t)V * G) return;
    const int g = (int)(i / V), v = (int)(i % V);
    int c[4] = {0, 0, 0, 0};
    for (int it = 1; it <= n; ++it) {
        const int idx = (int)((trace[(size_t)it * V + v] >> (2 * g)) & 3);
#pragma unroll
        for (int b = 0; b < 4; ++b) c[b] += (idx == b);
    }
    int64_t *p = out + ((size_t)v * G + g) * 4;
#pragma unroll
    for (int b = 0; b < 4; ++b) p[b] = c[b];
// ... 395 lines not shown
            p.sweep_stats[0] += (unsigned long long)red[0];
            p.sweep_stats[1] += (unsigned long long)redp[0];
            if (any_plain) { if (p.screen_ctl[0] > 0) p.screen_ctl[0] -= 1; }
            else if (5.0 * redp[0] > 4.0 * red[0]) p.screen_ctl[0] = 15;
        }
        if (p.blk_order) {
            __syncthreads();
            int *cnt = reinterpret_cast<int *>(red);
            const int per = (p.nblocks + nthr - 1) / nthr, lo = tid * per, hi = min(p.nblocks, lo + per);
            auto cold = [&](int i) { const uint32_t b = p.step_cnt[2 * i + 1]; return b != 0u && b != 0xFFFFFFFFu; };
            int nc = 0;
            for (int i = lo; i < hi; ++i) nc += cold(i) ? 1 : 0;
            int incl = nc;
            for (int o = 1; o < 64; o <<= 1) { const int y = __shfl_up(incl, o, 64); if ((tid & 63) >= o) incl += y; }
            if ((tid & 63) == 63) cnt[tid >> 6] = incl;
            __syncthreads();
            int before = incl - nc, total = 0;
            for (int k = 0; k < nthr / 64; ++k) { const int x = cnt[k]; if (k < (tid >> 6)) before += x; total += x; }
            int pc = before, pw = total + (lo - before);
            for (int i = lo; i < hi; ++i) { if (cold(i)) p.blk_order[pc++] = (uint32_t)i; else p.blk_order[pw++] = (uint32_t)i; }
        }
    }
}

__global__ __launch_bounds__(256) void finalize_kernel(FinalParams p)
{
    __shared__ double red[256], redp[256];
    __shared__ int flag;
    finalize_body(p, red, redp, &flag, threadIdx.x, 256);
    if (p.rare_out) {
        __syncthreads();
        if (threadIdx.x == 0) flag = 0;
        __syncthreads();
        for (int g = threadIdx.x; g < p.G; g += 256) {
            double m = 0.0;
            for (int s = 0; s < p.S; ++s) m = fmax(m, p.gamma_src[(size_t)s * p.G + g]);
            if ((float)m <= (float)DSM_NT_RARE) atomicAdd(&flag, 1);
        }
        __syncthreads();
        if (threadIdx.x == 0) *p.rare_out = flag;
    }
}

__device__ double gamma_variate(double shape, uint32_t idx, uint32_t iter, uint32_t k0, uint32_t k1)
{
    const double a = (shape < 1.0) ? shape + 1.0 : shape;
    const double d = a - 1.0 / 3.0;
    const double c = 1.0 / sqrt(9.0 * d);
    double res = 0.0, uboost = 1.0;
    for (uint32_t attempt = 0; attempt < 4096u; ++attempt) {
        uint32_t r0[4], r1[4];
        philox4x32_10(idx, 2u * attempt, iter, DSM_STREAM_DIRI, k0, k1, r0);
        philox4x32_10(idx, 2u * attempt + 1u, iter, DSM_STREAM_DIRI, k0, k1, r1);
        const double u1 = u01_open(r0[0], r0[1]), u2 = u01_open(r0[2], r0[3]);
        const double u3 = u01_open(r1[0], r1[1]);
        uboost = u01_open(r1[2], r1[3]);
        const double x = sqrt(-2.0 * log(u1)) * cos(6.283185307179586 * u2);
        double vv = 1.0 + c * x;
        if (vv <= 0.0) continue;
        vv = vv * vv * vv;
        const double x2 = x * x;
        if (u3 < 1.0 - 0.0331 * x2 * x2 || log(u3) < 0.5 * x2 + d * (1.0 - vv + log(vv))) {
            res = d * vv;
            break;
        }
    }
    if (shape < 1.0) res *= pow(uboost, 1.0 / shape);
    return res;
}

struct DirParams {
    unsigned long long *sum_mu, *esum;
    int S, G;
    double alpha, delta, epsilon, lgc_gamma, lgc_eta;
    uint32_t k0, k1, iter;
    int zero_after;
    double *gamma_out, *gamma_trace, *eta_out, *eta_trace, *rowprior;
    int do_fin;
    FinalParams fin;
    int do_s2;
    Stage2Params s2;
};

__device__ __forceinline__ void dirichlet_body(const DirParams &q, const S2Plan &plan)
{
    unsigned long long *__restrict__ sum_mu = q.sum_mu, *__restrict__ esum = q.esum;
    const int S = q.S, G = q.G;
    const double alpha = q.alpha, delta = q.delta, epsilon = q.epsilon, lgc_gamma = q.lgc_gamma, lgc_eta = q.lgc_eta;
    const uint32_t k0 = q.k0, k1 = q.k1, iter = q.iter;
    const int zero_after = q.zero_after;
    double *__restrict__ gamma_out = q.gamma_out, *__restrict__ gamma_trace = q.gamma_trace;
    double *__restrict__ eta_out = q.eta_out, *__restrict__ eta_trace = q.eta_trace, *__restrict__ rowprior = q.rowprior;
    const int do_fin = q.do_fin, do_s2 = q.do_s2;
    const FinalParams &fin = q.fin;
    const Stage2Params &s2 = q.s2;
    __shared__ __attribute__((aligned(16))) char smem_d[S2_SMEM_BYTES];
    if (do_fin && (int)blockIdx.x == S + 4) {
        double *red = reinterpret_cast<double *>(smem_d), *redp = red + 256;
        int *flag = reinterpret_cast<int *>(redp + 256);
        finalize_body(fin, red, redp, flag, threadIdx.x, 256);
        return;
    }
    const int row = blockIdx.x;
    const bool is_gamma = row < S;
    const uint32_t *leaf = nullptr;
    if (do_s2 && is_gamma)
        leaf = do_s2 >= 3 ? stage2_sample<3>(s2, plan, row, smem_d, false) : stage2_sample<2>(s2, plan, row, smem_d, false);
    if (!is_gamma) {
        static_assert(DSM_ESUM_PARTS * 4 == 256, "one thread per (copy, observed base)");
        unsigned long long *ef = reinterpret_cast<unsigned long long *>(smem_d);
        if (threadIdx.x < 4) ef[threadIdx.x] = 0ull;
        __syncthreads();
        const int ob = threadIdx.x & 3, k = threadIdx.x >> 2;
        unsigned long long *pp = esum + 16 + k * 16 + ob * 4 + (row - S);
        const unsigned long long v = *pp;
        if (v) { *pp = 0ull; atomicAdd(&ef[ob], v); }
        __syncthreads();
    }
    S2_CLK(row, 6);
    if (threadIdx.x >= 64) return;
    const int lane = threadIdx.x;
    const int n = is_gamma ? G : 4;
    const int SG = S * G;
    double y = 0.0;
    if (lane < n) {
        double shape;
        uint32_t vid;
        if (is_gamma) { vid = (uint32_t)(row * G + lane); shape = alpha + (double)(sum_mu[vid] + (leaf ? (unsigned long long)leaf[lane] : 0ull)); }
        else { const int a = row - S; vid = (uint32_t)(SG + a * 4 + lane); shape = delta + (double)(esum[lane * 4 + a] + reinterpret_cast<const unsigned long long *>(smem_d)[lane]); }
        y = gamma_variate(shape, vid, iter, k0, k1);
        if (zero_after) { if (is_gamma) sum_mu[row * G + lane] = 0ull; else esum[lane * 4 + (row - S)] = 0ull; }
    }
    double x = y / group_allreduce_sum<64>(y);
    if (is_gamma) {
        if (lane < n && x < epsilon) x = epsilon;
        x = x / group_allreduce_sum<64>(lane < n ? x : 0.0);
    }
    const double a1 = is_gamma ? alpha : delta;
    const double lsum = group_allreduce_sum<64>(lane < n ? (a1 - 1.0) * log(x) : 0.0);
    if (lane == 0) rowprior[row] = (is_gamma ? lgc_gamma : lgc_eta) + lsum;
    if (lane < n) {
        if (is_gamma) { gamma_out[row * G + lane] = x; if (gamma_trace) gamma_trace[row * G + lane] = x; }
        else { eta_out[(row - S) * 4 + lane] = x; if (eta_trace) eta_trace[(row - S) * 4 + lane] = x; }
    }
    S2_CLK(row, 7);
}
#ifdef DSM_AB_SWITCHES
extern "C" int dsm_debug_s2_clocks(unsigned long long *out, int nrows)
{
    if (nrows > 1024) nrows = 1024;
    if (hipMemcpyFromSymbol(out, HIP_SYMBOL(s2_clk), (size_t)nrows * 8 * sizeof(unsigned long long)) != hipSuccess) return -1;
    return 8;
}
#endif

struct DirBatch { DirParams p[DSM_MAX_BATCH]; S2Plan plan; };
__global__ __launch_bounds__(256) void dirichlet_kernel(DirParams q, S2Plan plan) { dirichlet_body(q, plan); }
__global__ __launch_bounds__(256) void dirichlet_kernel_b(DirBatch b) { dirichlet_body(b.p[blockIdx.y], b.plan); }
static_assert(sizeof(DirBatch) <= 4096, "kernarg segment");

__global__ __launch_bounds__(256) void prior_kernel(const double *__restrict__ gamma, const double *__restrict__ eta,
                                                    int S, int G, double alpha, double delta, double lgc_gamma,
                                                    double lgc_eta, double *__restrict__ rowprior)
{
    for (int r = blockIdx.x * 256 + threadIdx.x; r < S + 4; r += gridDim.x * 256) {
        double lsum = 0.0;
        if (r < S) { for (int g = 0; g < G; ++g) lsum += (alpha - 1.0) * log(gamma[(size_t)r * G + g]); rowprior[r] = lgc_gamma + lsum; }
        else { for (int b = 0; b < 4; ++b) lsum += (delta - 1.0) * log(eta[(r - S) * 4 + b]); rowprior[r] = lgc_eta + lsum; }
    }
}

struct TauParams {
    const int32_t *cnt_vs;
    uint64_t *tau;
    uint64_t *trace;
    const double *gamma, *eta_sweep, *eta_ll;
    const uint32_t *u_raw;
    double *logp;
    double *ll_partial;
    const double *log_tab;
    int *nchange;
    uint32_t *step_cnt;
    const uint32_t *screen_ctl;
    int screen;
    int nt_skip;
    int V, S, G;
    int v_off;
    uint32_t k0, k1, iter;
    const uint32_t *order;
    int do_fin;
    FinalParams fin;
};

#ifdef TAU_NO_LEAN
#define TAU_LEAN(LPV, NSL) false
#else
#ifdef TAU_LEAN2
#define TAU_LEAN(LPV, NSL) ((LPV) >= 32 && ((NSL) == 2 || (NSL) == 3 || (NSL) == 6 || (NSL) == 8))
#else
#define TAU_LEAN(LPV, NSL) ((LPV) >= 32 && ((NSL) == 3 || (NSL) == 6 || (NSL) == 8))
#endif
#endif

template <int LPV, int NSL, bool SWEEP, bool LL, bool NT = false>
__device__ __forceinline__ void tau_body(const TauParams &p)
{
    extern __shared__ __attribute__((aligned(16))) char smem_t[];
    const int nblk = (int)gridDim.x - p.do_fin;
    if (p.do_fin && (int)blockIdx.x == nblk) {
        double *fr = reinterpret_cast<double *>(smem_t);
        finalize_body(p.fin, fr, fr + 256, reinterpret_cast<int *>(fr + 512), threadIdx.x, 256);
        return;
    }
    constexpr bool LEAN = TAU_LEAN(LPV, NSL) && SWEEP;
    const int bid = p.order ? (int)p.order[blockIdx.x] : (int)blockIdx.x;
    constexpr int SP = LPV * NSL;
    constexpr int GPB = 256 / LPV;
    double *gT = reinterpret_cast<double *>(smem_t);
    double *eS = gT + (size_t)p.G * SP;
    double *eL = eS + 16;
    double *red = eL + 16;
    int *redi = reinterpret_cast<int *>(red + 4);
    double2 *ltab = reinterpret_cast<double2 *>(red + 6);
    float *gT32 = reinterpret_cast<float *>(ltab + DSM_LOG_TAB_N);
    float *eS32 = gT32 + (size_t)p.G * SP;
    uint32_t *gmaxb = reinterpret_cast<uint32_t *>(eS32 + 24);
    const int tid = threadIdx.x, G = p.G, S = p.S;
    if (tid < DSM_LOG_TAB_N) ltab[tid] = reinterpret_cast<const double2 *>(p.log_tab)[tid];
    if constexpr (NT) {
        if (tid < 32) gmaxb[tid] = 0u;
        __syncthreads();
    }
    for (int i = tid; i < G * SP; i += 256) {
        const int g = i / SP, s = i % SP;
        const double x = (s < S) ? p.gamma[(size_t)s * G + g] : 1.0;
        gT[i] = x;
        if (SWEEP) gT32[i] = (float)x;
        if constexpr (NT) { if (s < S && g < 32) atomicMax(&gmaxb[g], __float_as_uint((float)x)); }
    }
    if (tid < 16) { eS[tid] = p.eta_sweep[tid]; eL[tid] = p.eta_ll[tid]; if (SWEEP) eS32[tid] = (float)p.eta_sweep[tid]; }
    if (SWEEP && tid < 4) {
// ... 371 lines not shown
    const int key = gm * 2 + (exact ? 1 : 0);
    if (c->blk_gmax != key) {
        int occ = 0;
        HIP_TRY(hipOccupancyMaxActiveBlocksPerMultiprocessor(&occ, fn, 256, 0));
        hipDeviceProp_t prop;
        HIP_TRY(hipGetDeviceProperties(&prop, c->device));
        if (occ < 1) occ = 1;
        const int S = c->S, budget = std::max(S, occ * prop.multiProcessorCount);
        double tot = 0.0;
        for (int s = 0; s < S; ++s) tot += (double)c->depth[s];
        std::vector<int32_t> nb(S, 1);
        int used = S;
        if (tot > 0)
            for (int s = 0; s < S; ++s) {
                int extra = (int)((double)(budget - S) * (double)c->depth[s] / tot);
                const int most = (c->nitems_h[s] + 255) / 256;
                if (1 + extra > most) extra = std::max(0, most - 1);
                nb[s] += extra; used += extra;
            }
        std::vector<int32_t> tab;
        tab.reserve((size_t)used * 3);
        int maxnb = 0;
        for (int s = 0; s < S; ++s) maxnb = std::max(maxnb, nb[s]);
        for (int j = 0; j < maxnb; ++j)
            for (int s = 0; s < S; ++s)
                if (j < nb[s]) { tab.push_back(s); tab.push_back(j); tab.push_back(nb[s]); }
        if (c->blk_tab) { (void)hipFree(c->blk_tab); c->blk_tab = nullptr; }
        HIP_TRY(hipMalloc((void **)&c->blk_tab, tab.size() * sizeof(int32_t)));
        HIP_TRY(hipMemcpyAsync(c->blk_tab, tab.data(), tab.size() * sizeof(int32_t), hipMemcpyHostToDevice, c->stream));
        HIP_TRY(hipStreamSynchronize(c->stream));
        c->blk_n = used;
        c->blk_gmax = key;
    }
    const dim3 grid(c->blk_n), block(256);
    const uint32_t k0 = (uint32_t)c->ctr_seed, k1 = (uint32_t)(c->ctr_seed >> 32);
#define LAUNCH_STATS(GM, EX)                                                                                          \
    hipLaunchKernelGGL((stats_kernel<GM, EX>), grid, block, 0, c->stream, reinterpret_cast<const int2 *>(c->items),   \
                       c->nitems, c->blk_tab, c->tau, c->gamma, c->eta,                                               \
                       c->V, c->S, c->G, c->item_stride, c->chunked ? 1 : 0, k0, k1, iter, c->sum_mu, c->esum)
#define STATS_CASE(GM) if (gm == GM) { if (exact) LAUNCH_STATS(GM, true); else LAUNCH_STATS(GM, (GM <= 8)); }
    STATS_CASE(1); STATS_CASE(2); STATS_CASE(3); STATS_CASE(4); STATS_CASE(5); STATS_CASE(6); STATS_CASE(7);
    STATS_CASE(8); STATS_CASE(10); STATS_CASE(12); STATS_CASE(14); STATS_CASE(16); STATS_CASE(20); STATS_CASE(24);
    STATS_CASE(28); STATS_CASE(32);
#undef STATS_CASE
#undef LAUNCH_STATS
    HIP_TRY(hipGetLastError());
    return DSM_OK;
}

static void dirichlet_consts(const dsm_ctx *c, double *lgc_gamma, double *lgc_eta)
{
    *lgc_gamma = lgamma(c->alpha * c->G) - c->G * lgamma(c->alpha);
    *lgc_eta = lgamma(c->delta * 4) - 4 * lgamma(c->delta);
}

static FinalParams make_final(dsm_ctx *c, int nblocks, int it, int star_mode, const double *prior, const double *gamma_src,
                              const double *eta_src, int slot = 0)
{
    FinalParams p;
    p.ll_partial = c->ll_partial + (size_t)slot * DSM_MAX_GRID; p.nblocks = nblocks;
    p.ll_const = c->ll_const;
    p.tau_prior = (double)(c->shard_on ? c->shard_vtot : c->V) * (double)c->G * log(1.0 / 4.0);
    p.ll_given = c->shard_on ? c->shard_vec : nullptr;
    p.prior = prior; p.S = c->S; p.nchange = c->nchange + slot; p.it = it;
    p.ll_trace = c->ll_trace; p.lp_trace = c->lp_trace; p.nchange_trace = c->nchange_trace;
    p.star = c->star; p.gamma_src = gamma_src; p.gamma_star = c->gamma_star; p.SG = c->S * c->G;
    p.eta_src = eta_src; p.eta_star = c->eta_star;
    p.star_mode = star_mode; p.scalars = c->scalars;
    p.step_cnt = c->step_cnt + (size_t)slot * 2 * DSM_MAX_GRID; p.sweep_stats = c->sweep_stats; p.screen_ctl = c->screen_ctl + slot;
    static const bool order_on = !(getenv("DESMAN_HIP_TAU_ORDER") && atoi(getenv("DESMAN_HIP_TAU_ORDER")) == 0);
    p.blk_order = nullptr;
    p.rare_out = nullptr; p.G = c->G;
    if (order_on && c->blk_order && nblocks > 0 && nblocks <= DSM_MAX_GRID) {
        if (c->tau_resident_key != c->S * 64 + c->G) {
            int launched = 0, resident = 0;
            if (tau_launch_info(c, &launched, &resident) == DSM_OK) { c->tau_resident = resident; c->tau_resident_key = c->S * 64 + c->G; }
        }
        if (c->tau_resident > 0 && nblocks > c->tau_resident) { p.blk_order = c->blk_order + (size_t)slot * DSM_MAX_GRID; c->blk_order_n[slot] = nblocks; }
        else c->blk_order_n[slot] = 0;
    }
    return p;
}

int k_dirichlet(dsm_ctx *c, uint32_t iter, double *gamma_out, double *gamma_trace, double *eta_out, double *eta_trace,
                double *prior_out, int fin_it, int fin_nblocks, const double *fin_prior, int do_s2)
{
    KTimer tm(c, DSM_K_DIRICH);
    double lg, le;
    dirichlet_consts(c, &lg, &le);
    const uint32_t k0 = (uint32_t)c->ctr_seed, k1 = (uint32_t)(c->ctr_seed >> 32);
    const int do_fin = fin_it >= 0 ? 1 : 0;
    FinalParams fin = {};
    if (do_fin)
        fin = make_final(c, fin_nblocks, fin_it, 0, fin_prior, c->gamma_trace + (size_t)fin_it * c->S * c->G,
                         c->eta_trace + (size_t)fin_it * 16);
    Stage2Params s2 = {};
    if (do_s2) {
        s2.ntab = c->ntab; s2.rep = c->ntab_rep; s2.ld = c->ntab_ld; s2.gamma = c->gamma; s2.sum_mu = c->sum_mu; s2.log_tab = c->log_tab;
        s2.S = c->S; s2.G = c->G; s2.k0 = k0; s2.k1 = k1; s2.iter = iter; s2.hmul = DSM_NTAB_HMUL; s2.swz = DSM_NTAB_SWZ;
        s2.big_count = c->big_count;
    }
    DirParams q;
    q.sum_mu = c->sum_mu; q.esum = c->esum; q.S = c->S; q.G = c->G;
    q.alpha = c->alpha; q.delta = c->delta; q.epsilon = c->epsilon; q.lgc_gamma = lg; q.lgc_eta = le;
    q.k0 = k0; q.k1 = k1; q.iter = iter; q.zero_after = 1;
    q.gamma_out = gamma_out; q.gamma_trace = gamma_trace; q.eta_out = eta_out; q.eta_trace = eta_trace; q.rowprior = prior_out;
    q.do_fin = do_fin; q.fin = fin; q.do_s2 = do_s2 ? stats_draw_version(stats_spec(c)) : 0; q.s2 = s2;
    if (g_batch.K == 0) {
        const S2Plan plan = do_s2 ? make_stage2_plan(c->G) : S2Plan{};
        hipLaunchKernelGGL(dirichlet_kernel, dim3(c->S + 4 + do_fin), dim3(256), 0, c->stream, q, plan);
    } else {
        static thread_local DirBatch acc;
        acc.p[g_batch.k] = q;
        if (g_batch.k == g_batch.K - 1) {
            acc.plan = do_s2 ? make_stage2_plan(c->G) : S2Plan{};
            hipLaunchKernelGGL(dirichlet_kernel_b, dim3(c->S + 4 + do_fin, g_batch.K), dim3(256), 0, c->stream, acc);
        }
    }
    HIP_TRY(hipGetLastError());
    return DSM_OK;
}

__global__ __launch_bounds__(256) void prior_batch_kernel(const double *__restrict__ gamma, const double *__restrict__ eta,
                                                          int n, int S, int G, double alpha, double delta,
                                                          double lgc_gamma, double lgc_eta, double *__restrict__ rowprior)
{
    const int rows = S + 4;
    for (size_t i = (size_t)blockIdx.x * 256 + threadIdx.x; i < (size_t)n * rows; i += (size_t)gridDim.x * 256) {
        const int it = (int)(i / rows), r = (int)(i % rows);
        double lsum = 0.0;
        if (r < S) {
            const double *g = gamma + ((size_t)it * S + r) * G;
            for (int k = 0; k < G; ++k) lsum += (alpha - 1.0) * log(g[k]);
            rowprior[i] = lgc_gamma + lsum;
        } else {
            const double *e = eta + (size_t)it * 16 + (r - S) * 4;
            for (int b = 0; b < 4; ++b) lsum += (delta - 1.0) * log(e[b]);
            rowprior[i] = lgc_eta + lsum;
        }
    }
}

int k_prior_batch(dsm_ctx *c, const double *gamma, const double *eta, int n, double *prior_out)
{
    double lg, le;
    dirichlet_consts(c, &lg, &le);
    const size_t tot = (size_t)n * (c->S + 4);
    const int grid = (int)std::min<size_t>((tot + 255) / 256, 1024);
    hipLaunchKernelGGL(prior_batch_kernel, dim3(grid), dim3(256), 0, c->stream, gamma, eta, n, c->S, c->G, c->alpha, c->delta,
                       lg, le, prior_out);
    HIP_TRY(hipGetLastError());
    return DSM_OK;
}

int k_prior(dsm_ctx *c, const double *gamma, const double *eta, double *prior_out)
{
    double lg, le;
    dirichlet_consts(c, &lg, &le);
    hipLaunchKernelGGL(prior_kernel, dim3(1), dim3(256), 0, c->stream, gamma, eta, c->S, c->G, c->alpha, c->delta, lg,
                       le, prior_out);
    HIP_TRY(hipGetLastError());
    return DSM_OK;
}

__global__ __launch_bounds__(256) void gamma_rare_kernel(const double *__restrict__ gamma, int S, int G, int *__restrict__ out)
{
    __shared__ int cnt;
    if (threadIdx.x == 0) cnt = 0;
    __syncthreads();
    for (int g = threadIdx.x; g < G; g += 256) {
        double m = 0.0;
        for (int s = 0; s < S; ++s) m = fmax(m, gamma[(size_t)s * G + g]);
        if ((float)m <= (float)DSM_NT_RARE) atomicAdd(&cnt, 1);
    }
    __syncthreads();
    if (threadIdx.x == 0) *out = cnt;
}
int k_tau_neartie_hint(dsm_ctx *c)
{
    c->tau_neartie_on = false;
    if (c->tau_neartie_mode == 0 || g_batch.K || c->shard_on || !c->tau_screen || c->G < 2) return DSM_OK;
    c->tau_neartie_on = c->tau_neartie_mode == 1 || (c->tau_rare_n > 0 && c->tau_rare_n < c->G);
    return DSM_OK;
}
int tau_rare_from_host(const double *gamma, int S, int G)
{
    int n = 0;
    for (int g = 0; g < G; ++g) {
        double m = 0.0;
        for (int s = 0; s < S; ++s) m = std::max(m, gamma[(size_t)s * G + g]);
        n += (float)m <= (float)DSM_NT_RARE;
    }
    return n;
// ... 164 lines not shown
```

### desman_amd/csrc/kernels_stats.hip

```cpp
#include "dsm_binom.h"
#include "dsm_host.h"
#include "log_table.h"

#include <string.h>

#include <algorithm>
#include <vector>

#ifdef DSM_AB_SWITCHES
#define STATS_DBG(p, mask) ((p).dbg & (mask))
#else
#define STATS_DBG(p, mask) 0
#endif
#ifdef DSM_AB_SWITCHES
#define S1_NCLK 16
__device__ unsigned long long s1_clk[8192 * S1_NCLK];
#define S1_CLK(k) do { if ((threadIdx.x & 63) == 0 && blockIdx.y == 0) s1_clk[(size_t)(blockIdx.x * 4 + (threadIdx.x >> 6)) * S1_NCLK + (k)] = __builtin_amdgcn_s_memrealtime(); } while (0)
extern "C" int dsm_debug_s1_clocks(unsigned long long *out, int nwaves)
{
    if (nwaves > 8192) nwaves = 8192;
    if (hipMemcpyFromSymbol(out, HIP_SYMBOL(s1_clk), (size_t)nwaves * S1_NCLK * sizeof(unsigned long long)) != hipSuccess) return -1;
    return S1_NCLK;
}
#else
#define S1_CLK(k) do { } while (0)
#endif
#define S1_CLKP(j) do { if (s1_pass < 3) S1_CLK(2 + 4 * s1_pass + (j)); } while (0)
struct StatsAggParams {
    const int32_t *cnt_vs;
    const uint64_t *tau;
    const double *gamma, *eta;
    int V, S, G;
    int v_off, V_tot;
    uint32_t k0, k1, iter;
    uint32_t *ntab;
    int rep, ld;
    unsigned long long *esum;
    const double *log_tab;
    unsigned long long *big_list;
    uint32_t *big_count;
    size_t big_seg;
    double lean_cap;
    uint32_t swz;
    uint32_t hmul;
    int xcd;
    const unsigned long long *pat_rep;
    uint32_t *pat_x;
    const uint32_t *pat_list, *pat_n;
    int dbg;
};

__device__ __forceinline__ uint64_t wave_uniform_u64(uint64_t x)
{
    const uint32_t lo = __builtin_amdgcn_readfirstlane((uint32_t)x), hi = __builtin_amdgcn_readfirstlane((uint32_t)(x >> 32));
    return ((uint64_t)hi << 32) | lo;
}

template <int LPV, int SPEC, bool PAT = false>
__device__ __forceinline__ void stats_agg_body(const StatsAggParams &p)
{
    extern __shared__ __attribute__((aligned(16))) char smem_s[];
    S1_CLK(0);
#ifdef DSM_AB_SWITCHES
    if ((threadIdx.x & 63) == 0 && blockIdx.y == 0)
        s1_clk[(size_t)(blockIdx.x * 4 + (threadIdx.x >> 6)) * S1_NCLK + 13] =
            ((unsigned long long)(__builtin_amdgcn_s_getreg((31 << 11) | 4)) << 8) | (__builtin_amdgcn_s_getreg((3 << 11) | 20) & 15u) | (1ull << 63);
#endif
    constexpr int NG = 64 / LPV;
    constexpr int NTAB = SPEC >= 3 ? (2 * DSM_LOG_TAB_N + DSM_EXP_TAB_N) : 0;
    const int S = p.S, G = p.G, V = p.V;
    const int NCH = (S + LPV - 1) / LPV, SP = NCH * LPV;
    double *tabs = reinterpret_cast<double *>(smem_s);
    double *gT = tabs + NTAB;
    double *rcp = gT + (size_t)G * SP;
    double *es = rcp + DSM_RCP_TAB_N;
    uint32_t *eacc = reinterpret_cast<uint32_t *>(es + 16);
    const double2 *ltab = reinterpret_cast<const double2 *>(tabs);
    const int tid = threadIdx.x, lane = tid & 63;
    const int grp = lane / LPV, lig = lane % LPV;
    const int nwaves = gridDim.x * 4;
    const int wid = __builtin_amdgcn_readfirstlane(blockIdx.x * 4 + (tid >> 6));
    const int nunit = PAT ? (int)__builtin_amdgcn_readfirstlane((int)*p.pat_n) : V;
// ... 186 lines not shown
{
    const int v = blockIdx.x * 256 + threadIdx.x;
    if (v >= V) return;
    atomicMin(&rep[tau[v] & ((1ull << (2 * G)) - 1ull)], ((unsigned long long)hi << 32) | (unsigned long long)(uint32_t)v);
}
__global__ __launch_bounds__(1024) void pat_rep_lds_kernel(const uint64_t *__restrict__ tau, int V, int G, unsigned long long *__restrict__ rep, uint32_t hi)
{
    __shared__ uint32_t lo[4096];
    const int words = 1 << (2 * G), tid = threadIdx.x;
    for (int i = tid; i < words; i += 1024) lo[i] = 0xFFFFFFFFu;
    __syncthreads();
    const uint64_t mask = (1ull << (2 * G)) - 1ull;
    for (int v = blockIdx.x * 1024 + tid; v < V; v += gridDim.x * 1024) atomicMin(&lo[tau[v] & mask], (uint32_t)v);
    __syncthreads();
    for (int i = tid; i < words; i += 1024)
        if (lo[i] != 0xFFFFFFFFu) atomicMin(&rep[i], ((unsigned long long)hi << 32) | (unsigned long long)lo[i]);
}
template <int LPW>
__global__ __launch_bounds__(1024) void pat_agg_lds_kernel(const int32_t *__restrict__ cnt_vs, const uint64_t *__restrict__ tau, int V, int S, int G,
                                                           const unsigned long long *__restrict__ rep, uint32_t *__restrict__ x, int nvsplit)
{
    extern __shared__ uint32_t ptab[];
    const int words = 1 << (2 * G);
    const int tid = threadIdx.x, lane = tid & 63, wv = tid >> 6;
    for (int i = tid; i < words * 4 * LPW; i += 1024) ptab[i] = 0u;
    __syncthreads();
    constexpr int PPW = 64 / LPW;
    const int chunk = (int)blockIdx.x / nvsplit, part = (int)blockIdx.x % nvsplit;
    const int s = chunk * LPW + (lane % LPW);
    const uint64_t mask = (1ull << (2 * G)) - 1ull;
    for (int v0 = (part * 16 + wv) * PPW; v0 < V; v0 += nvsplit * 16 * PPW) {
        const int v = v0 + lane / LPW;
        if (v < V && s < S) {
            const int4 c = reinterpret_cast<const int4 *>(cnt_vs)[(size_t)v * S + s];
            uint32_t *row = ptab + (size_t)(tau[v] & mask) * 4 * LPW + (lane % LPW);
            if (c.x) atomicAdd(row, (uint32_t)c.x);
            if (c.y) atomicAdd(row + LPW, (uint32_t)c.y);
            if (c.z) atomicAdd(row + 2 * LPW, (uint32_t)c.z);
            if (c.w) atomicAdd(row + 3 * LPW, (uint32_t)c.w);
        }
    }
    __syncthreads();
    for (int i = tid; i < words * 4 * LPW; i += 1024) {
        const uint32_t n = ptab[i];
        if (!n) continue;
        const int w = i / (4 * LPW), b = (i / LPW) & 3, sl = chunk * LPW + i % LPW;
        atomicAdd(x + ((size_t)(uint32_t)rep[w] * 4 + b) * S + sl, n);
    }
}

__global__ __launch_bounds__(256) void pat_list_kernel(const unsigned long long *__restrict__ rep, int words, uint32_t hi, uint32_t *__restrict__ list,
                                                       uint32_t *__restrict__ n_this, uint32_t *__restrict__ n_next)
{
    const int w = blockIdx.x * 256 + threadIdx.x;
    if (w == 0) *n_next = 0u;
    if (w >= words) return;
    const unsigned long long e = rep[w];
    if ((uint32_t)(e >> 32) == hi) list[atomicAdd(n_this, 1u)] = (uint32_t)e;
}

__global__ __launch_bounds__(256) void pat_agg_kernel(const int32_t *__restrict__ cnt_vs, const uint64_t *__restrict__ tau, int V, int S, int G,
                                                      const unsigned long long *__restrict__ rep, uint32_t *__restrict__ x)
{
    const size_t n = (size_t)V * S;
    for (size_t i = (size_t)blockIdx.x * 256 + threadIdx.x; i < n; i += (size_t)gridDim.x * 256) {
        const int v = (int)(i / (size_t)S), s = (int)(i - (size_t)v * S);
        const int4 c = reinterpret_cast<const int4 *>(cnt_vs)[i];
        const uint32_t r = (uint32_t)rep[tau[v] & ((1ull << (2 * G)) - 1ull)];
        uint32_t *xr = x + (size_t)r * 4 * S + s;
        if (c.x) atomicAdd(xr, (uint32_t)c.x);
        if (c.y) atomicAdd(xr + S, (uint32_t)c.y);
        if (c.z) atomicAdd(xr + 2 * (size_t)S, (uint32_t)c.z);
        if (c.w) atomicAdd(xr + 3 * (size_t)S, (uint32_t)c.w);
    }
}
template <int LPV, int SPEC>
__global__ __launch_bounds__(256, 6) void stats_agg_kernel_b(BatchArgs<StatsAggParams> b) { stats_agg_body<LPV, SPEC>(b.p[blockIdx.y]); }
template <int LPV>
__global__ __launch_bounds__(256, 5) void stats_pat_kernel_b(BatchArgs<StatsAggParams> b) { stats_agg_body<LPV, 2, true>(b.p[blockIdx.y]); }

template <int SPEC>
__device__ __forceinline__ void stats_big_body(const StatsAggParams &p)
{
    __shared__ double2 ltab[DSM_LOG_TAB_N + DSM_EXP_TAB_N / 2];
    __shared__ double rcp[DSM_RCP_TAB_N];
    __shared__ double es[16];
    __shared__ unsigned long long acc[16];
    __shared__ uint32_t eacc[16 * 256];
    const int tid = threadIdx.x, lane = tid & 63;
    const uint32_t sub = blockIdx.x % (DSM_BIG_NT * DSM_BIG_NL), bi = blockIdx.x / (DSM_BIG_NT * DSM_BIG_NL), nb = gridDim.x / (DSM_BIG_NT * DSM_BIG_NL);
    const uint32_t nbig = p.big_count[sub * DSM_BIG_STRIDE];
    if (bi * 256u >= nbig) return;
    const unsigned long long *list = p.big_list + (size_t)sub * p.big_seg;
    ltab[tid] = reinterpret_cast<const double2 *>(p.log_tab)[tid];
    if (tid < DSM_EXP_TAB_N / 2) ltab[DSM_LOG_TAB_N + tid] = reinterpret_cast<const double2 *>(p.log_tab)[DSM_LOG_TAB_N + tid];
    for (int k = tid; k < DSM_RCP_TAB_N; k += blockDim.x) rcp[k] = k ? 1.0 / (double)k : 0.0;
    if (tid < 16) { es[tid] = p.eta[tid]; acc[tid] = 0ull; }
#pragma unroll
    for (int i = 0; i < 16; ++i) eacc[i * 256 + tid] = 0u;
    __syncthreads();
    const int S = p.S, G = p.G;
    for (uint32_t i = bi * 256u + tid; i < nbig; i += nb * 256u) {
        const unsigned long long item = list[i];
        const uint32_t cell = (uint32_t)(item >> 2);
        const int b = (int)(item & 3ull);
        const int s = (int)(cell / (uint32_t)p.V_tot), v = (int)(cell - (uint32_t)s * (uint32_t)p.V_tot) - p.v_off;
        const uint64_t t = p.tau[v];
        uint32_t xb;
        if (p.pat_x) { uint32_t *xw = p.pat_x + ((size_t)v * 4 + b) * S + s; xb = *xw; *xw = 0u; }
        else xb = (uint32_t)p.cnt_vs[((size_t)v * S + s) * 4 + b];
        uint32_t H[4] = {0, 0, 0, 0};
        double Gam[4] = {0.0, 0.0, 0.0, 0.0};
        for (int g = 0; g < G; ++g) {
            const int a = (int)((t >> (2 * g)) & 3);
            const double x = p.gamma[(size_t)s * G + g];
#pragma unroll
            for (int k = 0; k < 4; ++k) if (a == k) { H[k] |= 1u << g; Gam[k] = Gam[k] + x; }
        }
        double W[4];
#pragma unroll
        for (int a = 0; a < 4; ++a) W[a] = es[a * 4 + b] * Gam[a];
        const double Wt = ((W[0] + W[1]) + W[2]) + W[3];
        if (!(Wt > 0.0)) {
#pragma unroll
            for (int a = 0; a < 4; ++a) W[a] = Gam[a];
        }
        uint32_t n[4], cbase[4];
        philox4x32_10(cell, 0u, p.iter, DSM_STREAM_STA1, p.k0, p.k1, cbase);
        Xo128 rng = item_seed<SPEC>(cbase, (uint32_t)b, p.k0, p.k1);
        bool defer = false;
        mult4<true, SPEC>(rng, xb, W, n, rcp, ltab, defer);
        uint32_t *erow = eacc + (b * 4) * 256 + tid;
#pragma unroll
        for (int a = 0; a < 4; ++a) {
            erow[a * 256] += n[a];
            if (n[a]) atomicAdd(p.ntab + (size_t)(blockIdx.x % (unsigned)p.rep) * (((size_t)1 << G) * (size_t)p.ld) + (size_t)((H[a] * p.hmul + ((uint32_t)s >> 4) * p.swz) & ((1u << G) - 1u)) * (size_t)p.ld + s, n[a]);
        }
    }
    {
        uint32_t e[16];
#pragma unroll
        for (int i = 0; i < 16; ++i) e[i] = eacc[i * 256 + tid];
        const uint32_t tot = wave_transpose_reduce<16>(e);
        const int idx = transpose_index<16>(lane);
        if (lane < 16 && tot) atomicAdd(&acc[idx], (unsigned long long)tot);
    }
    __syncthreads();
    if (tid < 16 && acc[tid]) atomicAdd(&p.esum[tid], acc[tid]);
}

__global__ __launch_bounds__(256) void esum_fold_kernel(unsigned long long *__restrict__ esum)
{
    static_assert(DSM_ESUM_PARTS * 4 == 256, "one thread per (copy, group of four counters)");
    const int k = threadIdx.x >> 2, q = threadIdx.x & 3;
    unsigned long long *pp = esum + 16 + k * 16 + q * 4;
#pragma unroll
    for (int i = 0; i < 4; ++i) {
        const unsigned long long v = pp[i];
        if (v) { pp[i] = 0ull; atomicAdd(&esum[q * 4 + i], v); }
    }
}
int k_esum_fold(dsm_ctx *c)
{
    hipLaunchKernelGGL(esum_fold_kernel, dim3(1), dim3(256), 0, c->stream, c->esum);
    HIP_TRY(hipGetLastError());
    return DSM_OK;
}

template <int SPEC>
__global__ __launch_bounds__(256) void stats_big_kernel(StatsAggParams p) { stats_big_body<SPEC>(p); }
template <int SPEC>
__global__ __launch_bounds__(256) void stats_big_kernel_b(BatchArgs<StatsAggParams> b) { stats_big_body<SPEC>(b.p[blockIdx.y]); }

#include "dsm_stage2.h"

struct Stage2Batch { Stage2Params p[DSM_MAX_BATCH]; S2Plan plan; };
template <int SPEC>
__global__ __launch_bounds__(1024) void stats_stage2_kernel(Stage2Params p, S2Plan plan)
{
    __shared__ __attribute__((aligned(16))) char smem2[S2_SMEM_BYTES];
    stage2_sample<SPEC>(p, plan, (int)blockIdx.x / p.nsplit, smem2, true, (int)blockIdx.x % p.nsplit);
}
template <int SPEC>
__global__ __launch_bounds__(1024) void stats_stage2_kernel_b(Stage2Batch b)
{
    __shared__ __attribute__((aligned(16))) char smem2[S2_SMEM_BYTES];
    stage2_sample<SPEC>(b.p[blockIdx.y], b.plan, blockIdx.x, smem2, true);
}

template <int SPEC>
__global__ __launch_bounds__(256) void binom_test_kernel(int kind, uint32_t n, double wa, double wb, double w2, double w3,
                                                         uint32_t k0, uint32_t k1, int nsamp, const double *log_tab,
                                                         uint32_t *out)
{
    __shared__ double2 ltab[DSM_LOG_TAB_N + DSM_EXP_TAB_N / 2];
    __shared__ double rcp[DSM_RCP_TAB_N];
    const int tid = threadIdx.x;
    ltab[tid] = reinterpret_cast<const double2 *>(log_tab)[tid];
    if (tid < DSM_EXP_TAB_N / 2) ltab[DSM_LOG_TAB_N + tid] = reinterpret_cast<const double2 *>(log_tab)[DSM_LOG_TAB_N + tid];
    for (int k = tid; k < DSM_RCP_TAB_N; k += blockDim.x) rcp[k] = k ? 1.0 / (double)k : 0.0;
    __syncthreads();
    const int i = blockIdx.x * 256 + tid;
    if (i >= nsamp) return;
    Xo128 rng = xo_seed((uint32_t)i, 0u, 0u, DSM_STREAM_TEST, k0, k1);
    bool dummy = false;
    if (kind != 2) out[i] = binom<true, SPEC>(rng, n, wa, wb, rcp, ltab, dummy, kind == 0 ? DSM_BINV_MEAN_CAP : DSM_BINV_MEAN_CAP_S2);
    else {
        const double W[4] = {wa, wb, w2, w3};
        uint32_t m[4];
        mult4<true, SPEC>(rng, n, W, m, rcp, ltab, dummy);
        out[i * 4 + 0] = m[0]; out[i * 4 + 1] = m[1]; out[i * 4 + 2] = m[2]; out[i * 4 + 3] = m[3];
    }
}

static int stats_agg_lpv(int S)
{
    int best = 64;
    for (int l : {32, 16}) if ((S + l - 1) / l * l < (S + best - 1) / best * best) best = l;
    return best;
}

int stats_spec(const dsm_ctx *c)
{
    int force = c->force_stats_spec;
    if (force == 0) {
        const char *e = getenv("DESMAN_HIP_STATS_SPEC");
        if (e && (e[0] == '1' || e[0] == '2' || e[0] == '3' || e[0] == '4') && e[1] == 0) force = e[0] - '0';
    }
    if (force == 1) return 1;
    if (c->G < 1 || c->G > 16) return 1;
    if (((size_t)1 << c->G) * (size_t)c->S * 4 > ((size_t)64 << 20)) return 1;
    if (c->max_depth >= ((uint64_t)1 << 32)) return 1;
    const bool pat_ok = c->G <= 8 && !c->shard_on;
    if (force == 4) return pat_ok ? 4 : 2;
    if (force >= 2) return force;
    double reads = 0.0;
    for (int64_t d : c->depth) reads += (double)d;
    const int lpv = stats_agg_lpv(c->S);
    const double cells = (double)c->V * (double)((c->S + lpv - 1) / lpv * lpv);
    const double g = (double)c->G;
    const double t1 = 25.0 + (0.25 + 0.02 * g + 0.0029 * g * g) * 1e-6 * reads;
    const double stage2 = 14.0 + (c->G >= 10 ? 0.012 * (double)(1u << c->G) : 0.0);
    const int rep = stats_ntab_rep(c);
    const double per = 3.0 * (double)c->V / (double)(1u << c->G);
    const double t2 = 24.0 + stage2 + 0.062e-3 * cells + (rep == 1 ? 0.03 * per : 0.003 * per / rep);
    if (pat_ok && force == 0 && t2 < t1) {
        const bool small_g = (c->G <= 2 && cells >= 0.5e6) || (c->G == 3 && cells >= 1.0e6);
        const bool mid_g = c->G >= 4 && cells >= 2.5e6 && 64.0 * (double)((size_t)1 << c->G) <= (double)c->V;
        if (small_g || mid_g) return 4;
    }
    return t2 < t1 ? DSM_STATS_AGG : 1;
}

int stats_ntab_rep(const dsm_ctx *c)
{
    const double per = 3.0 * (double)(c->shard_on ? c->shard_vtot : c->V) / (double)((size_t)1 << c->G);
    if (per <= 128.0) return 1;
    const double lines = (double)((((size_t)1 << c->G) * (size_t)c->S * 4 + 63) / 64);
    int rep = 2;
    while (lines * rep < 384.0 && rep < 64 && (size_t)(2 * rep) * ((size_t)1 << c->G) * (size_t)c->S * 4 <= ((size_t)64 << 20)) rep *= 2;
    return rep;
}

void stats_release_ntab(dsm_ctx *c)
{
    if (c->ntab_raw) (void)hipFree(c->ntab_raw);
    c->ntab_raw = nullptr; c->ntab = nullptr; c->ntab_len = 0;
}
static int ensure_ntab(dsm_ctx *c)
{
    const int rep = stats_ntab_rep(c), ld = c->S;
    const size_t need = (size_t)rep * ((size_t)1 << c->G) * (size_t)ld;
    if (c->ntab && c->ntab_len == need && c->ntab_ld == ld && c->ntab_rep == rep) return DSM_OK;
    stats_release_ntab(c);
    c->ntab_rep = rep; c->ntab_ld = ld;
    const char *eo = DSM_AB_ENV("DESMAN_HIP_NTAB_OFF");
    const size_t off = eo ? ((size_t)strtoull(eo, nullptr, 0) & ~(size_t)255) : 0;
    const size_t spare = off + 4096;
    hipError_t e = hipMalloc((void **)&c->ntab_raw, need * sizeof(uint32_t) + spare);
    if (e != hipSuccess) { dsm_set_error("hipMalloc(%zu B) failed: %s", need * 4 + spare, hipGetErrorString(e)); return DSM_ERR_NOMEM; }
    c->ntab = reinterpret_cast<uint32_t *>(((uintptr_t)c->ntab_raw + 4095) & ~(uintptr_t)4095) + off / 4;
    c->ntab_len = need;
    HIP_TRY(hipMemsetAsync(c->ntab, 0, need * sizeof(uint32_t), c->stream));
    return DSM_OK;
}

int stats_ensure_ntab(dsm_ctx *c)
{
    return stats_spec(c) < 2 ? DSM_OK : ensure_ntab(c);
}

static int ensure_big_list(dsm_ctx *c, size_t seg)
{
    const size_t need = seg * DSM_BIG_NT * DSM_BIG_NL;
    if (c->big_list && c->big_cap == need) return DSM_OK;
    if (c->big_list) { (void)hipFree(c->big_list); c->big_list = nullptr; }
    if (!c->big_count) {
        hipError_t e = hipMalloc((void **)&c->big_count, DSM_BIG_NT * DSM_BIG_NL * DSM_BIG_STRIDE * sizeof(uint32_t));
        if (e != hipSuccess) { dsm_set_error("hipMalloc failed: %s", hipGetErrorString(e)); return DSM_ERR_NOMEM; }
    }
    hipError_t e = hipMalloc((void **)&c->big_list, need * sizeof(unsigned long long));
    if (e != hipSuccess) { dsm_set_error("hipMalloc(%zu B) failed: %s", need * 8, hipGetErrorString(e)); return DSM_ERR_NOMEM; }
    c->big_cap = need;
    HIP_TRY(hipMemsetAsync(c->big_count, 0, DSM_BIG_NT * DSM_BIG_NL * DSM_BIG_STRIDE * sizeof(uint32_t), c->stream));
    return DSM_OK;
}

static int ensure_pat(dsm_ctx *c)
{
    const size_t nrep = (size_t)1 << (2 * c->G), nx = (size_t)c->V * 4 * (size_t)c->S;
    if (!c->pat_rep || c->pat_rep_len != nrep) {
        if (c->pat_rep) { (void)hipFree(c->pat_rep); c->pat_rep = nullptr; }
        hipError_t e = hipMalloc((void **)&c->pat_rep, nrep * sizeof(unsigned long long));
        if (e != hipSuccess) { dsm_set_error("hipMalloc(%zu B) failed: %s", nrep * 8, hipGetErrorString(e)); return DSM_ERR_NOMEM; }
        c->pat_rep_len = nrep;
        c->pat_gen = 0;
        HIP_TRY(hipMemsetAsync(c->pat_rep, 0xFF, nrep * sizeof(unsigned long long), c->stream));
    }
    if (!c->pat_list || c->pat_rep_len != nrep || c->pat_gen == 0) {
        if (c->pat_list) { (void)hipFree(c->pat_list); c->pat_list = nullptr; }
        hipError_t e = hipMalloc((void **)&c->pat_list, (nrep + 2) * sizeof(uint32_t));
        if (e != hipSuccess) { dsm_set_error("hipMalloc(%zu B) failed: %s", (nrep + 2) * 4, hipGetErrorString(e)); return DSM_ERR_NOMEM; }
        HIP_TRY(hipMemsetAsync(c->pat_list + nrep, 0, 2 * sizeof(uint32_t), c->stream));
    }
    if (!c->pat_x || c->pat_x_len != nx) {
        if (c->pat_x) { (void)hipFree(c->pat_x); c->pat_x = nullptr; }
        hipError_t e = hipMalloc((void **)&c->pat_x, nx * sizeof(uint32_t));
        if (e != hipSuccess) { dsm_set_error("hipMalloc(%zu B) failed: %s", nx * 4, hipGetErrorString(e)); return DSM_ERR_NOMEM; }
        c->pat_x_len = nx;
        HIP_TRY(hipMemsetAsync(c->pat_x, 0, nx * sizeof(uint32_t), c->stream));
    }
    return DSM_OK;
}

int k_stats_stage1(dsm_ctx *c, uint32_t iter)
{
    int r = ensure_ntab(c);
    if (r != DSM_OK) return r;
    const int S = c->S, G = c->G, V = c->V;
    const int LPV = stats_agg_lpv(S);
    const int NCH = (S + LPV - 1) / LPV, SP = NCH * LPV, NG = 64 / LPV;
    const int spec_full = stats_spec(c);
    const bool pat = spec_full == 4;
    const int spec = stats_draw_version(spec_full);
    const size_t sh = ((size_t)G * SP + (spec >= 3 ? 2 * DSM_LOG_TAB_N + DSM_EXP_TAB_N : 0) + DSM_RCP_TAB_N + 16) * sizeof(double) +
                      16 * 256 * sizeof(uint32_t);
    if (sh > 160 * 1024) { dsm_set_error("stats_agg: gamma tile (%zu B) exceeds LDS", sh); return DSM_ERR_UNSUPPORTED; }
    const void *fn = nullptr, *fn_b = nullptr;
#define AGG_CASE(L, SP_) if (LPV == L && spec == SP_) { fn = (const void *)stats_agg_kernel<L, SP_>; fn_b = (const void *)stats_agg_kernel_b<L, SP_>; }
    AGG_CASE(16, 2) AGG_CASE(32, 2) AGG_CASE(64, 2) AGG_CASE(16, 3) AGG_CASE(32, 3) AGG_CASE(64, 3)
#undef AGG_CASE
    if (pat) {
        fn = LPV == 16 ? (const void *)stats_pat_kernel<16> : LPV == 32 ? (const void *)stats_pat_kernel<32> : (const void *)stats_pat_kernel<64>;
        fn_b = LPV == 16 ? (const void *)stats_pat_kernel_b<16> : LPV == 32 ? (const void *)stats_pat_kernel_b<32> : (const void *)stats_pat_kernel_b<64>;
    }
    if (!fn) { dsm_set_error("stats_agg: no kernel for spec %d", spec); return DSM_ERR_UNSUPPORTED; }
    if (c->stats_grid == 0 || c->stats_grid_key != spec_full) {
        int occ = 0;
        HIP_TRY(hipOccupancyMaxActiveBlocksPerMultiprocessor(&occ, fn, 256, sh));
        hipDeviceProp_t prop;
        HIP_TRY(hipGetDeviceProperties(&prop, c->device));
        const int wgs = std::min(6, std::max(1, occ));
        const int n_xcd = prop.multiProcessorCount % 8 == 0 && prop.multiProcessorCount >= 64 ? 8 : 1;
        const long passes4 = (((long)V * NCH + NG - 1) / NG) / std::max(1L, (long)wgs * prop.multiProcessorCount);
        const int leave = (c->tau_rng == DSM_RNG_MT19937 && passes4 <= 12) ? n_xcd : 0;
        c->stats_grid = wgs * std::max(1, prop.multiProcessorCount - leave);
        c->stats_grid_key = spec_full;
    }
    const long ntask = ((long)V * NCH + NG - 1) / NG;
    const long max_waves = (long)c->stats_grid * 4 / (g_batch.K ? g_batch.K : 1);
    const long waves = std::min<long>(ntask, max_waves);
    const int grid = (int)std::max<long>(1, (waves + 3) / 4);
    const long per_wg = ((ntask + waves - 1) / waves) * 4 * 64 * 4;
    const size_t seg = (size_t)std::min<long>((long)V * S * 4, ((grid + DSM_BIG_NL - 1) / DSM_BIG_NL) * per_wg);
    r = ensure_big_list(c, seg);
    if (r != DSM_OK) return r;
    StatsAggParams p;
    p.cnt_vs = c->cnt_vs; p.tau = c->tau; p.gamma = c->gamma; p.eta = c->eta;
    p.V = V; p.S = S; p.G = G; p.big_seg = seg;
    p.v_off = c->shard_on ? c->shard_voff : 0; p.V_tot = c->shard_on ? c->shard_vtot : V;
    p.k0 = (uint32_t)c->ctr_seed; p.k1 = (uint32_t)(c->ctr_seed >> 32); p.iter = iter;
    p.ntab = c->ntab; p.rep = c->ntab_rep; p.ld = c->ntab_ld; p.esum = c->esum; p.log_tab = c->log_tab;
    p.xcd = 0;
    p.hmul = DSM_NTAB_HMUL; p.swz = DSM_NTAB_SWZ;
    p.big_list = c->big_list; p.big_count = c->big_count;
    p.pat_rep = nullptr; p.pat_x = nullptr; p.pat_list = nullptr; p.pat_n = nullptr;
    if (pat) {
        r = ensure_pat(c);
        if (r != DSM_OK) return r;
        p.pat_rep = c->pat_rep; p.pat_x = c->pat_x;
        KTimer tm(c, DSM_K_STATSPAT);
        const uint32_t hi = 0xFFFFFFFFu - (++c->pat_gen);
        const int words = 1 << (2 * G);
        uint32_t *n_this = c->pat_list + words + (c->pat_gen & 1u), *n_next = c->pat_list + words + ((c->pat_gen + 1u) & 1u);
        p.pat_list = c->pat_list; p.pat_n = n_this;
        if (G <= 6) hipLaunchKernelGGL(pat_rep_lds_kernel, dim3(std::max(1, std::min(64, V / 4096))), dim3(1024), 0, c->stream, c->tau, V, G, c->pat_rep, hi);
        else hipLaunchKernelGGL(pat_rep_kernel, dim3((V + 255) / 256), dim3(256), 0, c->stream, c->tau, V, G, c->pat_rep, hi);
        hipLaunchKernelGGL(pat_list_kernel, dim3((words + 255) / 256), dim3(256), 0, c->stream, c->pat_rep, words, hi, c->pat_list, n_this, n_next);
        const size_t ncell = (size_t)V * S;
        const int lpw = G <= 3 ? 64 : 32;
        const size_t lds = ((size_t)1 << (2 * G)) * 4 * lpw * sizeof(uint32_t);
        if (G <= 4 && lds <= 128 * 1024 && V >= 4096) {
            const int nchunk = (S + lpw - 1) / lpw;
            const int nvsplit = std::max(1, std::min(256 / nchunk, V / (16 * (64 / lpw) * 8)));
            const void *fl = lpw == 64 ? (const void *)pat_agg_lds_kernel<64> : (const void *)pat_agg_lds_kernel<32>;
            static bool attr_done[2] = {false, false};
            if (!attr_done[lpw == 32]) { HIP_TRY(hipFuncSetAttribute(fl, hipFuncAttributeMaxDynamicSharedMemorySize, 128 * 1024)); attr_done[lpw == 32] = true; }
            const int32_t *cv = c->cnt_vs; const uint64_t *tp = c->tau; const unsigned long long *rp = c->pat_rep; uint32_t *xp = c->pat_x;
            int Vv = V, Ss = S, Gg = G, nvs = nvsplit;
            void *args[] = {(void *)&cv, (void *)&tp, (void *)&Vv, (void *)&Ss, (void *)&Gg, (void *)&rp, (void *)&xp, (void *)&nvs};
            HIP_TRY(hipLaunchKernel(fl, dim3(nchunk * nvsplit), dim3(1024), args, lds, c->stream));
        } else
            hipLaunchKernelGGL(pat_agg_kernel, dim3((unsigned)std::min<size_t>((ncell + 255) / 256, 16384)), dim3(256), 0, c->stream,
                               c->cnt_vs, c->tau, V, S, G, c->pat_rep, c->pat_x);
        HIP_TRY(hipGetLastError());
    }
    {
        static const char *e = DSM_AB_ENV("DESMAN_HIP_LEAN_CAP");
        p.lean_cap = e ? atof(e) : DSM_LEAN_CAP;
        static const int dbg = DSM_AB_ENV("DESMAN_HIP_STATS_DBG") ? atoi(DSM_AB_ENV("DESMAN_HIP_STATS_DBG")) : 0;
        p.dbg = dbg;
        if (!(p.lean_cap > 0.0 && p.lean_cap <= DSM_BINV_MEAN_CAP)) p.lean_cap = DSM_LEAN_CAP;
    }
    const int big_wgs = 16;
    const int big_grid = DSM_BIG_NT * DSM_BIG_NL *
        (int)std::max<long>(1, std::min<long>((ntask * 64 * 4 / DSM_BIG_NL + 255) / 256, g_batch.K ? std::max(2, big_wgs / g_batch.K) : big_wgs));
    if (g_batch.K) {
        static thread_local BatchArgs<StatsAggParams> acc;
        acc.p[g_batch.k] = p;
        if (g_batch.k == g_batch.K - 1) {
            const dim3 g(grid, g_batch.K);
            void *args[] = {(void *)&acc};
            HIP_TRY(hipLaunchKernel(fn_b, g, dim3(256), args, sh, c->stream));
            if (spec >= 3) hipLaunchKernelGGL(stats_big_kernel_b<3>, dim3(big_grid, g_batch.K), dim3(256), 0, c->stream, acc);
            else hipLaunchKernelGGL(stats_big_kernel_b<2>, dim3(big_grid, g_batch.K), dim3(256), 0, c->stream, acc);
        }
        HIP_TRY(hipGetLastError());
        return DSM_OK;
    }
    {
        KTimer tm(c, DSM_K_STATS);
        void *args[] = {(void *)&p};
        HIP_TRY(hipLaunchKernel(fn, dim3(grid), dim3(256), args, sh, c->stream));
    }
    KTimer tm(c, DSM_K_STATSBIG);
    if (spec >= 3) hipLaunchKernelGGL(stats_big_kernel<3>, dim3(big_grid), dim3(256), 0, c->stream, p);
    else hipLaunchKernelGGL(stats_big_kernel<2>, dim3(big_grid), dim3(256), 0, c->stream, p);
    HIP_TRY(hipGetLastError());
    return DSM_OK;
}

S2Plan make_stage2_plan(int G)
{
    S2Plan pl;
    memset(&pl, 0, sizeof pl);
    int n = 0, off = 0;
    pl.lo[0] = 0; pl.hi[0] = G; pl.off[0] = 0; pl.idx[0] = 0; pl.child[0] = -1;
    n = 1;
    int lvl_begin = 0, lvl_end = 1, level = 0;
    pl.level_start[0] = 0;
    while (lvl_begin < lvl_end) {
        for (int i = lvl_begin; i < lvl_end; ++i) {
            const int w = pl.hi[i] - pl.lo[i];
            if (w == 1) { pl.child[i] = -1; continue; }
            const int wl = w / 2, mid = pl.lo[i] + wl;
            pl.child[i] = n;
            pl.lo[n] = pl.lo[i]; pl.hi[n] = mid; pl.off[n] = off; pl.idx[n] = 2 * pl.idx[i]; off += 1 << wl; ++n;
            pl.lo[n] = mid; pl.hi[n] = pl.hi[i]; pl.off[n] = off; pl.idx[n] = 2 * pl.idx[i] + 1; off += 1 << (w - wl); ++n;
        }
        lvl_begin = lvl_end; lvl_end = n;
        pl.level_start[++level] = lvl_begin;
    }
    pl.nlevels = level;
    pl.tab_entries = off;
    return pl;
}

int k_stats_stage2(dsm_ctx *c, uint32_t iter)
{
    KTimer tm(c, DSM_K_STATS2);
    Stage2Params p;
    p.ntab = c->ntab; p.rep = c->ntab_rep; p.ld = c->ntab_ld; p.gamma = c->gamma; p.sum_mu = c->sum_mu; p.log_tab = c->log_tab;
    p.S = c->S; p.G = c->G; p.hmul = DSM_NTAB_HMUL; p.swz = DSM_NTAB_SWZ;
    p.k0 = (uint32_t)c->ctr_seed; p.k1 = (uint32_t)(c->ctr_seed >> 32); p.iter = iter;
    p.big_count = c->big_count;
    const int nthr = c->G >= 10 ? 1024 : 256;
    const bool v3 = stats_draw_version(stats_spec(c)) >= 3;
    p.nsplit = 1; p.scratch = nullptr; p.ticket = nullptr;
    if (g_batch.K == 0 && c->G >= 11) {
        if (!c->s2_scratch) {
            hipError_t e = hipMalloc((void **)&c->s2_scratch, ((size_t)DSM_MAX_S * (S2_TAB_ENTRIES + 1)) * sizeof(uint32_t));
            if (e != hipSuccess) { dsm_set_error("hipMalloc failed: %s", hipGetErrorString(e)); return DSM_ERR_NOMEM; }
            HIP_TRY(hipMemsetAsync(c->s2_scratch, 0, ((size_t)DSM_MAX_S * (S2_TAB_ENTRIES + 1)) * sizeof(uint32_t), c->stream));
        }
        p.nsplit = c->G >= 12 ? 4 : 2;
        p.scratch = c->s2_scratch; p.ticket = c->s2_scratch + (size_t)DSM_MAX_S * S2_TAB_ENTRIES;
    }
    if (g_batch.K == 0) {
        if (v3) hipLaunchKernelGGL(stats_stage2_kernel<3>, dim3(c->S * p.nsplit), dim3(nthr), 0, c->stream, p, make_stage2_plan(c->G));
        else hipLaunchKernelGGL(stats_stage2_kernel<2>, dim3(c->S * p.nsplit), dim3(nthr), 0, c->stream, p, make_stage2_plan(c->G));
    } else {
        static thread_local Stage2Batch acc;
        acc.p[g_batch.k] = p;
        if (g_batch.k == g_batch.K - 1) {
            acc.plan = make_stage2_plan(c->G);
            if (v3) hipLaunchKernelGGL(stats_stage2_kernel_b<3>, dim3(c->S, g_batch.K), dim3(nthr), 0, c->stream, acc);
            else hipLaunchKernelGGL(stats_stage2_kernel_b<2>, dim3(c->S, g_batch.K), dim3(nthr), 0, c->stream, acc);
        }
    }
    HIP_TRY(hipGetLastError());
    return DSM_OK;
}

int k_stats(dsm_ctx *c, uint32_t iter)
{
    if (stats_spec(c) >= 2) {
        int r = k_stats_stage1(c, iter);
        if (r != DSM_OK) return r;
        return k_stats_stage2(c, iter);
    }
    return k_stats_v1(c, iter);
}

int k_binom_test(dsm_ctx *c, int kind, uint32_t n, const double *w, uint64_t seed, int nsamp, uint32_t *d_out, int spec)
{
    if (spec >= 3) hipLaunchKernelGGL(binom_test_kernel<3>, dim3((nsamp + 255) / 256), dim3(256), 0, c->stream, kind, n, w[0], w[1], w[2], w[3],
                                      (uint32_t)seed, (uint32_t)(seed >> 32), nsamp, c->log_tab, d_out);
// ... 6 lines not shown
```

### include/desman_hip.h

```cpp
#ifndef DESMAN_HIP_H
#define DESMAN_HIP_H

#include <stdint.h>

#ifdef __cplusplus
extern "C" {
#endif

#define DSM_OK               0
#define DSM_ERR_HIP         -1
#define DSM_ERR_ARG         -2
#define DSM_ERR_STATE       -3
#define DSM_ERR_UNSUPPORTED -4
#define DSM_ERR_NOMEM       -5
#define DSM_ERR_NODEVICE    -6
#define DSM_ERR_COMM        -7

#define DSM_MAX_G  32
#define DSM_MAX_S  512

#define DSM_RNG_MT19937 0
#define DSM_RNG_PHILOX  1

const char *dsm_last_error(void);
int dsm_device_count(void);
const char *dsm_version(void);

int dsm_initRNG(void);
int dsm_setRNG(unsigned long seed);
int dsm_freeRNG(void);
int dsm_sample_tau(int64_t *tau, const double *pi, const double *eta,
                   const int64_t *variants, int nV, int nG, int nS);
void c_initRNG(void);
void c_setRNG(unsigned long seed);
void c_freeRNG(void);
int c_sample_tau(long *tau, double *pi, double *eta, long *variants, int nV, int nG, int nS);
int dsm_getRNG_state(uint32_t *state625);
int dsm_setRNG_state(const uint32_t *state625);

typedef struct dsm_ctx dsm_ctx;

int dsm_ctx_create(dsm_ctx **out, int device);
int dsm_ctx_destroy(dsm_ctx *ctx);
int dsm_ctx_sync(dsm_ctx *ctx);

int dsm_ctx_set_counts(dsm_ctx *ctx, const int64_t *variants, int V, int S);

int dsm_ctx_set_state(dsm_ctx *ctx, const int64_t *tau, const double *gamma,
                      const double *eta, int G);
int dsm_ctx_get_state(dsm_ctx *ctx, int64_t *tau, double *gamma, double *eta);
int dsm_ctx_set_gamma_eta(dsm_ctx *ctx, const double *gamma, const double *eta);

int dsm_ctx_set_priors(dsm_ctx *ctx, double alpha, double delta, double epsilon);

int dsm_ctx_seed(dsm_ctx *ctx, unsigned long mt_seed, uint64_t ctr_seed);
int dsm_ctx_set_tau_rng(dsm_ctx *ctx, int mode );
int dsm_ctx_get_mt_state(dsm_ctx *ctx, uint32_t *state625);
int dsm_ctx_set_mt_state(dsm_ctx *ctx, const uint32_t *state625);
int dsm_ctx_debug_mt_fill(dsm_ctx *ctx, size_t n, uint32_t *out);
int dsm_mt_seed_state(unsigned long seed, uint32_t *state625);

int dsm_ctx_sample_tau(dsm_ctx *ctx, int *nchange, double *logp_out);

int dsm_ctx_sample_stats(dsm_ctx *ctx, uint32_t iter, uint64_t *sum_mu, uint64_t *esum);
int dsm_ctx_stats_spec(dsm_ctx *ctx);
int dsm_ctx_force_stats_spec(dsm_ctx *ctx, int spec);
int dsm_ctx_debug_stage1(dsm_ctx *ctx, uint32_t iter, uint32_t *ntab, uint64_t *esum);
int dsm_ctx_debug_binom(dsm_ctx *ctx, int kind, uint32_t n, const double *w4, uint64_t seed, int nsamp,
                        uint32_t *out, int spec);

int dsm_ctx_draw_gamma_eta(dsm_ctx *ctx, uint32_t iter, const uint64_t *sum_mu,
                           const uint64_t *esum, double *gamma_out, double *eta_out);

int dsm_ctx_loglik(dsm_ctx *ctx, double *ll, double *lp);

int dsm_ctx_gibbs_update(dsm_ctx *ctx, int n_iter);
int dsm_batch_gibbs_update(dsm_ctx *const *ctxs, int n_ctx, int n_iter);
int dsm_ctx_update_tau(dsm_ctx *ctx, int n_iter, const double *gamma_store,
                       const double *eta_store);
int dsm_batch_update_tau(dsm_ctx *const *ctxs, int n_ctx, int n_iter, const double *const *gamma_stores,
                         const double *const *eta_stores);

int dsm_ctx_get_trace(dsm_ctx *ctx, double *ll, double *lp, int32_t *nchange,
                      double *gamma_store, double *eta_store);
int dsm_ctx_get_star(dsm_ctx *ctx, int64_t *tau_star, double *gamma_star,
                     double *eta_star, double *lp_star, int *iter_star);
int dsm_ctx_get_tau_sum(dsm_ctx *ctx, int64_t *tau_sum);
int dsm_ctx_get_tau_at(dsm_ctx *ctx, int it, int64_t *tau);

int dsm_nmft_set(dsm_ctx *ctx, const double *tau, const double *gamma, int G);
int dsm_nmft_get(dsm_ctx *ctx, double *tau, double *gamma);
int dsm_nmft_factorize(dsm_ctx *ctx, int max_iter, double min_change, int fix_gamma,
                       int *n_done, double *div_trace);
int dsm_batch_nmft_factorize(dsm_ctx *const *ctxs, int n_ctx, int max_iter, double min_change, int fix_gamma,
                             int *n_done, double *div_traces);
int dsm_nmft_objective(dsm_ctx *ctx, double *div);
int dsm_nmft_get_tau(dsm_ctx *ctx, int64_t *tau_onehot);

int dsm_lrt_step(int device, const double *ffreq, const int32_t *maxA, const int32_t *maxB,
                 const double *eta, double upperP, int optimise, int V, double *p_inout,
                 double *MLL, double *BLL);

#define DSM_ASSIGN_MAX_G 10
int dsm_assign_tau(int device, const int64_t *counts , int N, int S, int G, const double *gamma, const double *eta,
                   uint64_t seed, uint8_t *map_state, double *conf, double *logz, double *marg, uint8_t *draw_state);
int dsm_ctx_assign_tau(dsm_ctx *ctx, const double *gamma, const double *eta, int G, uint64_t seed, uint8_t *map_state,
                       double *conf, double *logz, double *marg, uint8_t *draw_state);
int dsm_assign_debug_set_chunk(int positions);

typedef struct dsm_genes dsm_genes;
#define DSM_MAX_ETA 8

int dsm_genes_create(dsm_genes **out, int device);
int dsm_genes_destroy(dsm_genes *gs);
int dsm_genes_set_data(dsm_genes *gs, const int64_t *variants, int Vtot, int S, int C,
                       const int32_t *gene_off , const double *cov);
int dsm_genes_set_model(dsm_genes *gs, const double *gamma, const double *epsilon,
                        const double *delta, int G, int max_eta, const double *eta_log_prior,
                        const double *cov_const, const double *mult_const);
int dsm_genes_set_state(dsm_genes *gs, const int32_t *eta, const int64_t *tau);
int dsm_genes_get_state(dsm_genes *gs, int32_t *eta, int64_t *tau);
int dsm_genes_seed(dsm_genes *gs, unsigned long mt_seed, uint64_t ctr_seed);
int dsm_genes_set_gene_base(dsm_genes *gs, int gene_base);
int dsm_genes_get_mt_state(dsm_genes *gs, uint32_t *state625);
int dsm_genes_set_mt_state(dsm_genes *gs, const uint32_t *state625);

int dsm_genes_nmft_tau(dsm_genes *gs, const int32_t *eta_mask ,
                       const double *tau_init, int max_iter, double min_change, int32_t *n_iter);
int dsm_genes_sweep_all(dsm_genes *gs, const int32_t *eta_mask, int sweep, int32_t *nchange,
                        double *logvar, double *v_ll);
int dsm_genes_step_candidates(dsm_genes *gs, int c, int g, double *logvar, int *swept);
int dsm_genes_step_choose(dsm_genes *gs, int c, int g, int eta_value);
int dsm_genes_update(dsm_genes *gs, int n_iter, int reset_star, int32_t *eta_store,
                     double *gene_ll_trace, const uint32_t *u_tau_ext, const double *u_eta_ext);
int dsm_genes_loglik(dsm_genes *gs, double *gene_ll);
int dsm_genes_get_star(dsm_genes *gs, int32_t *eta_star, double *gene_llstar);
int dsm_genes_set_star(dsm_genes *gs, const int32_t *eta_star, const double *gene_llstar);

int dsm_kl_assign(int device, const double *cov, const double *delta, double *eta, int C, int S,
                  int G, int max_iter, double min_change, int *n_done, double *div);

#define DSM_K_STATS    0
#define DSM_K_DIRICH   1
#define DSM_K_TAU      2
#define DSM_K_FINAL    3
#define DSM_K_MT       4
#define DSM_K_NMFT_A   5
#define DSM_K_NMFT_G   6
#define DSM_K_NMFT_B   7
#define DSM_K_STATS2   8
// ... 40 lines not shown
```

Measured before the change: 6.317 billion V*S updates/s.

## Fold deferred big-item stats draws into the Dirichlet launch with a grid barrier

Moves the stage-1 big-item multinomial draws out of their own kernel launch and into extra helper workgroups of the fused Dirichlet/stage-2 kernel. The helpers meet the rest of the grid at a software barrier before stage 2 reads the tables. This removes one kernel launch per Gibbs iteration. In exchange it depends on every workgroup being co-resident, adds a spin barrier with a timeout/error path that voids the chain, and raises LDS use in the Dirichlet kernel.

Result: faster. 6.384 billion V*S updates/s (median of 6 runs) (+1.1%).

```diff
diff --git a/desman_amd/_lib.py b/desman_amd/_lib.py
--- a/desman_amd/_lib.py
+++ b/desman_amd/_lib.py
@@ -67,6 +67,8 @@
     "dsm_release_device_caches": (_i, []),
     "dsm_ctx_force_stats_spec": (_i, [_vp, _i]),
     "dsm_ctx_debug_stage1": (_i, [_vp, C.c_uint32, _vp, _u64p]),
+    "dsm_ctx_debug_deferred_drawn": (_i, [_vp, _vp]),
+    "dsm_ctx_set_deferred_inlaunch": (_i, [_vp, _i]),
     "dsm_ctx_debug_binom": (_i, [_vp, _i, C.c_uint32, _f64p, C.c_uint64, _i, _u32p, _i]),
     "dsm_ctx_draw_gamma_eta": (_i, [_vp, C.c_uint32, _u64p, _u64p, _f64p, _f64p]),
     "dsm_ctx_loglik": (_i, [_vp, C.POINTER(_d), C.POINTER(_d)]),
@@ -414,6 +416,14 @@
         check(self.lib.dsm_ctx_debug_stage1(self._h, int(it), nt.ctypes.data, E))
         return nt, E
 
+    def debug_deferred_drawn(self):
+        n = C.c_uint64(0)
+        check(self.lib.dsm_ctx_debug_deferred_drawn(self._h, C.byref(n)))
+        return int(n.value)
+
+    def set_deferred_inlaunch(self, mode=-1):
+        check(self.lib.dsm_ctx_set_deferred_inlaunch(self._h, int(mode)))
+
     def debug_binom(self, kind, n, w, seed, nsamp, spec=STATS_AGG):
         w4 = np.zeros(4)
         w4[:len(w)] = w
diff --git a/desman_amd/csrc/api.hip b/desman_amd/csrc/api.hip
--- a/desman_amd/csrc/api.hip
+++ b/desman_amd/csrc/api.hip
@@ -219,7 +219,8 @@
     dev_free(&c->pat_rep); dev_free(&c->pat_x); dev_free(&c->pat_list); c->pat_rep_len = c->pat_x_len = 0;
     if (c->h_rare) { (void)hipHostFree(c->h_rare); c->h_rare = nullptr; }
     dev_free(&c->s2_scratch);
-    dev_free(&c->blk_tab); stats_release_ntab(c); dev_free(&c->big_list); dev_free(&c->big_count);
+    dev_free(&c->blk_tab); stats_release_ntab(c); dev_free(&c->big_list); dev_free(&c->big_count); dev_free(&c->big_bar);
+    if (c->h_big_err) { (void)hipHostFree(c->h_big_err); c->h_big_err = nullptr; }
     dev_free(&c->gamma); dev_free(&c->eta);
     dev_free(&c->eta_new); dev_free(&c->sum_mu); dev_free(&c->esum); dev_free(&c->mt_state); dev_free(&c->mt_jstates); dev_free(&c->u_raw);
     dev_free(&c->ll_partial); dev_free(&c->nchange); dev_free(&c->sweep_stats); dev_free(&c->step_cnt); dev_free(&c->blk_order); dev_free(&c->screen_ctl); dev_free(&c->prior); dev_free(&c->prior_all); dev_free(&c->scalars); dev_free(&c->star);
@@ -279,6 +280,7 @@
     c->max_items = 0;
     c->blk_gmax = 0;
     c->stats_grid = 0;
+    c->big_helpers_key = -1;
     dev_free(&c->pat_x); c->pat_x_len = 0;
     TRY(reset_blk_order(c));
     HIP_TRY(hipMemsetAsync(c->screen_ctl, 0, 4 * sizeof(uint32_t), c->stream));
@@ -372,6 +374,7 @@
         TRY(dev_alloc(&c->sum_mu, sg));
         HIP_TRY(hipMemsetAsync(c->sum_mu, 0, sg * sizeof(unsigned long long), c->stream));
         c->stats_grid = 0;
+    c->big_helpers_key = -1;
         c->u_cap = (size_t)c->V * G;
         c->u_chunk_words = c->u_cap * std::max<size_t>(1, std::min<size_t>(DSM_U_CHUNK, ((size_t)16 << 20) / std::max<size_t>(1, c->u_cap)));
         TRY(dev_alloc(&c->u_raw, 2 * c->u_chunk_words));
@@ -681,6 +684,16 @@
                 for (int r = 0; r < c->ntab_rep; ++r) v += t[((size_t)r * NH + ((h * DSM_NTAB_HMUL + (s >> 4) * DSM_NTAB_SWZ) & (NH - 1))) * ld + s];
                 ntab[s * NH + h] = v;
             }
+    return DSM_OK;
+}
+
+extern "C" int dsm_ctx_debug_deferred_drawn(dsm_ctx *c, uint64_t *drawn)
+{
+    if (!c || !drawn) { dsm_set_error("debug_deferred_drawn: bad arguments"); return DSM_ERR_ARG; }
+    BIND(c);
+    *drawn = 0;
+    HIP_TRY(hipStreamSynchronize(c->stream));
+    if (c->big_bar) HIP_TRY(hipMemcpy(drawn, c->big_bar + DSM_BIGBAR_DRAWN, sizeof(uint64_t), hipMemcpyDeviceToHost));
     return DSM_OK;
 }
 
@@ -834,6 +847,7 @@
     const int spec = stats_spec(lead);
     const bool agg = spec >= 2;
     const bool fuse_s2 = agg && lead->G < 10;
+    const int big_helpers = (fuse_s2 && !batched) ? dirichlet_big_helpers(lead) : -1;
     const size_t sg = (size_t)lead->S * lead->G;
     std::vector<SweepWords> words;
     words.reserve(K);
@@ -852,11 +866,11 @@
     TRY(ch.launch([&](dsm_ctx *, int k) { return words[k].prefetch(); }));
     for (int it = 0; it < n_iter; ++it) {
         if (!batched && it && (it & 63) == 0 && lead->tau_neartie_mode == -1) { TRY(k_tau_rare_count(lead, true)); TRY(k_tau_neartie_hint(lead)); }
-        TRY(ch.launch([&](dsm_ctx *c, int k) { ic[k] = c->iter_ctr++; return agg ? k_stats_stage1(c, ic[k]) : k_stats_v1(c, ic[k]); }));
+        TRY(ch.launch([&](dsm_ctx *c, int k) { ic[k] = c->iter_ctr++; return agg ? k_stats_stage1(c, ic[k], big_helpers >= 0) : k_stats_v1(c, ic[k]); }));
         if (agg && !fuse_s2) TRY(ch.launch([&](dsm_ctx *c, int k) { return k_stats_stage2(c, ic[k]); }));
         TRY(ch.launch([&](dsm_ctx *c, int k) {
             return k_dirichlet(c, ic[k], c->gamma, c->gamma_trace + (size_t)it * sg, c->eta_new, c->eta_trace + (size_t)it * 16,
-                               prior_slot(c, it), it - 1, nb_prev[k], prior_slot(c, it - 1), fuse_s2 ? 1 : 0);
+                               prior_slot(c, it), it - 1, nb_prev[k], prior_slot(c, it - 1), fuse_s2 ? 1 : 0, big_helpers);
         }));
         TRY(ch.launch([&](dsm_ctx *, int k) { return words[k].acquire(it, &u[k]); }));
         TRY(ch.launch([&](dsm_ctx *c, int k) {
@@ -875,8 +889,21 @@
             return k_finalize(c, nb_prev[k], n_iter - 1, 0, prior_slot(c, n_iter - 1), c->gamma_trace + (size_t)(n_iter - 1) * sg,
                               c->eta_trace + (size_t)(n_iter - 1) * 16, 0, want_rare ? c->h_rare : nullptr);
         }));
+    const bool big_used = big_helpers >= 0 && n_iter > 0 && lead->big_bar;
+    if (big_used) {
+        if (!lead->h_big_err) HIP_TRY(hipHostMalloc((void **)&lead->h_big_err, sizeof(unsigned), hipHostMallocDefault));
+        HIP_TRY(hipMemcpyAsync(lead->h_big_err, lead->big_bar + DSM_BIGBAR_ERR, sizeof(unsigned), hipMemcpyDeviceToHost, lead->stream));
+    }
     HIP_TRY(hipStreamSynchronize(lead->stream));
     if (want_rare) lead->tau_rare_n = *lead->h_rare;
+    if (big_used && *lead->h_big_err) {
+        HIP_TRY(hipMemsetAsync(lead->big_bar, 0, (DSM_BIGBAR_DRAWN) * sizeof(unsigned), lead->stream));
+        HIP_TRY(hipMemsetAsync(lead->big_count, 0, DSM_BIG_NT * DSM_BIG_NL * DSM_BIG_STRIDE * sizeof(uint32_t), lead->stream));
+        HIP_TRY(hipStreamSynchronize(lead->stream));
+        lead->big_helpers = -1;
+        dsm_set_error("gibbs_update: the workgroups of a Dirichlet launch did not meet at its barrier (deferred stage-1 items); the chain's state is void");
+        return DSM_ERR_STATE;
+    }
     return DSM_OK;
 }
 
@@ -1078,6 +1105,14 @@
 {
     if (!c || mode < -1 || mode > 3 || mode == 2) { dsm_set_error("set_nmft_fused: mode -1, 0, 1 or 3"); return DSM_ERR_ARG; }
     c->nmft_fused = mode;
+    return DSM_OK;
+}
+
+extern "C" int dsm_ctx_set_deferred_inlaunch(dsm_ctx *c, int mode)
+{
+    if (!c || mode < -1 || mode > 1) { dsm_set_error("set_deferred_inlaunch: -1 (by the table's depth), 0 or 1"); return DSM_ERR_ARG; }
+    c->big_inlaunch_mode = mode;
+    c->big_helpers_key = -1;
     return DSM_OK;
 }
 
diff --git a/desman_amd/csrc/dsm_big.h b/desman_amd/csrc/dsm_big.h
--- /dev/null
+++ b/desman_amd/csrc/dsm_big.h
@@ -0,0 +1,175 @@
+#pragma once
+#include "dsm_binom.h"
+#include "dsm_host.h"
+#include "log_table.h"
+
+struct BigParams {
+    const int32_t *cnt_vs;
+    const uint64_t *tau;
+    const double *gamma, *eta;
+    int S, G, v_off, V_tot;
+    uint32_t k0, k1, iter;
+    uint32_t *ntab;
+    int rep, ld;
+    unsigned long long *esum;
+    const double *log_tab;
+    const unsigned long long *big_list;
+    uint32_t *big_count;
+    size_t big_seg;
+    uint32_t swz, hmul;
+    uint32_t *pat_x;
+    unsigned *bar;
+};
+
+#define DSM_BIG_SMEM_BYTES ((DSM_LOG_TAB_N + DSM_EXP_TAB_N / 2) * 16 + DSM_RCP_TAB_N * 8 + 16 * 8 + 16 * 8 + 16 * 256 * 4)
+struct BigLds { double2 *ltab; double *rcp, *es; unsigned long long *acc; uint32_t *eacc; };
+
+__device__ __forceinline__ BigLds big_lds(char *smem)
+{
+    BigLds l;
+    l.ltab = reinterpret_cast<double2 *>(smem);
+    l.rcp = reinterpret_cast<double *>(l.ltab + DSM_LOG_TAB_N + DSM_EXP_TAB_N / 2);
+    l.es = l.rcp + DSM_RCP_TAB_N;
+    l.acc = reinterpret_cast<unsigned long long *>(l.es + 16);
+    l.eacc = reinterpret_cast<uint32_t *>(l.acc + 16);
+    return l;
+}
+
+template <class P>
+__device__ __forceinline__ void big_begin(const P &p, const BigLds &l)
+{
+    const int tid = threadIdx.x;
+    l.ltab[tid] = reinterpret_cast<const double2 *>(p.log_tab)[tid];
+    if (tid < DSM_EXP_TAB_N / 2) l.ltab[DSM_LOG_TAB_N + tid] = reinterpret_cast<const double2 *>(p.log_tab)[DSM_LOG_TAB_N + tid];
+    for (int k = tid; k < DSM_RCP_TAB_N; k += 256) l.rcp[k] = k ? 1.0 / (double)k : 0.0;
+    if (tid < 16) { l.es[tid] = p.eta[tid]; l.acc[tid] = 0ull; }
+#pragma unroll
+    for (int i = 0; i < 16; ++i) l.eacc[i * 256 + tid] = 0u;
+    __syncthreads();
+}
+
+template <int SPEC, class P>
+__device__ __forceinline__ void big_item(const P &p, const BigLds &l, unsigned long long item, uint32_t copy)
+{
+    const int tid = threadIdx.x;
+    const int S = p.S, G = p.G;
+    const uint32_t cell = (uint32_t)(item >> 2);
+    const int b = (int)(item & 3ull);
+    const int s = (int)(cell / (uint32_t)p.V_tot), v = (int)(cell - (uint32_t)s * (uint32_t)p.V_tot) - p.v_off;
+    const uint64_t t = p.tau[v];
+    uint32_t xb;
+    if (p.pat_x) { uint32_t *xw = p.pat_x + ((size_t)v * 4 + b) * S + s; xb = *xw; *xw = 0u; }
+    else xb = (uint32_t)p.cnt_vs[((size_t)v * S + s) * 4 + b];
+    uint32_t H[4] = {0, 0, 0, 0};
+    double Gam[4] = {0.0, 0.0, 0.0, 0.0};
+    for (int g = 0; g < G; ++g) {
+        const int a = (int)((t >> (2 * g)) & 3);
+        const double x = p.gamma[(size_t)s * G + g];
+#pragma unroll
+        for (int k = 0; k < 4; ++k) if (a == k) { H[k] |= 1u << g; Gam[k] = Gam[k] + x; }
+    }
+    double W[4];
+#pragma unroll
+    for (int a = 0; a < 4; ++a) W[a] = l.es[a * 4 + b] * Gam[a];
+    const double Wt = ((W[0] + W[1]) + W[2]) + W[3];
+    if (!(Wt > 0.0)) {
+#pragma unroll
+        for (int a = 0; a < 4; ++a) W[a] = Gam[a];
+    }
+    uint32_t n[4], cbase[4];
+    philox4x32_10(cell, 0u, p.iter, DSM_STREAM_STA1, p.k0, p.k1, cbase);
+    Xo128 rng = item_seed<SPEC>(cbase, (uint32_t)b, p.k0, p.k1);
+    bool defer = false;
+    mult4<true, SPEC>(rng, xb, W, n, l.rcp, l.ltab, defer);
+    uint32_t *erow = l.eacc + (b * 4) * 256 + tid;
+#pragma unroll
+    for (int a = 0; a < 4; ++a) {
+        erow[a * 256] += n[a];
+        if (n[a]) atomicAdd(p.ntab + (size_t)copy * (((size_t)1 << G) * (size_t)p.ld) + (size_t)((H[a] * p.hmul + ((uint32_t)s >> 4) * p.swz) & ((1u << G) - 1u)) * (size_t)p.ld + s, n[a]);
+    }
+}
+
+template <class P>
+__device__ __forceinline__ void big_end(const P &p, const BigLds &l)
+{
+    const int tid = threadIdx.x, lane = tid & 63;
+    {
+        uint32_t e[16];
+#pragma unroll
+        for (int i = 0; i < 16; ++i) e[i] = l.eacc[i * 256 + tid];
+        const uint32_t tot = wave_transpose_reduce<16>(e);
+        const int idx = transpose_index<16>(lane);
+        if (lane < 16 && tot) atomicAdd(&l.acc[idx], (unsigned long long)tot);
+    }
+    __syncthreads();
+    if (tid < 16 && l.acc[tid]) atomicAdd(&p.esum[tid], l.acc[tid]);
+}
+
+#define DSM_BIG_INL_SMEM_BYTES (DSM_BIG_SMEM_BYTES + DSM_BIG_NT * DSM_BIG_NL * 4 + 16)
+
+typedef __attribute__((address_space(1))) unsigned big_gu32;
+#define BIG_RLX_AGENT __ATOMIC_RELAXED, __HIP_MEMORY_SCOPE_AGENT
+
+__device__ __forceinline__ bool big_grid_barrier(unsigned *bar, unsigned members, int *ok_s)
+{
+    asm volatile("s_waitcnt vmcnt(0)" ::: "memory");
+    __syncthreads();
+    if (threadIdx.x == 0) {
+        int ok = 1;
+        big_gu32 *cnt = (big_gu32 *)(bar + DSM_BIGBAR_CNT), *gen = (big_gu32 *)(bar + DSM_BIGBAR_GEN), *err = (big_gu32 *)(bar + DSM_BIGBAR_ERR);
+        const unsigned g0 = __hip_atomic_load(gen, BIG_RLX_AGENT);
+        __builtin_amdgcn_fence(__ATOMIC_RELEASE, "agent");
+        asm volatile("s_waitcnt vmcnt(0)" ::: "memory");
+        const unsigned t = __hip_atomic_fetch_add(cnt, 1u, BIG_RLX_AGENT);
+        if (t + 1u == members) {
+            __hip_atomic_store(cnt, 0u, BIG_RLX_AGENT);
+            __hip_atomic_store(gen, g0 + 1u, BIG_RLX_AGENT);
+        } else {
+            unsigned spins = 0;
+            while (__hip_atomic_load(gen, BIG_RLX_AGENT) == g0) {
+                __builtin_amdgcn_s_sleep(2);
+                if (__hip_atomic_load(err, BIG_RLX_AGENT) != 0u || ++spins > (1u << 22)) {
+                    __hip_atomic_store(err, 1u, BIG_RLX_AGENT);
+                    ok = 0;
+                    break;
+                }
+            }
+        }
+        __builtin_amdgcn_fence(__ATOMIC_ACQUIRE, "agent");
+        asm volatile("s_waitcnt vmcnt(0)" ::: "memory");
+        *ok_s = ok;
+    }
+    __syncthreads();
+    return *ok_s != 0;
+}
+
+template <int SPEC>
+__device__ __forceinline__ bool big_inlaunch(const BigParams &p, char *smem, uint32_t n_mine, uint32_t member, uint32_t members)
+{
+    constexpr int NLIST = DSM_BIG_NT * DSM_BIG_NL;
+    const int tid = threadIdx.x;
+    const BigLds l = big_lds(smem);
+    uint32_t *cnt_s = reinterpret_cast<uint32_t *>(smem + DSM_BIG_SMEM_BYTES);
+    int *ok_s = reinterpret_cast<int *>(cnt_s + NLIST);
+    if (tid < NLIST) cnt_s[tid] = n_mine;
+    big_begin(p, l);
+    uint32_t base = 0, next = member;
+    for (int sub = 0; sub < NLIST; ++sub) {
+        const uint32_t nbig = cnt_s[sub], nchunk = (nbig + 255u) / 256u;
+        const unsigned long long *list = p.big_list + (size_t)sub * p.big_seg;
+        for (; next < base + nchunk; next += members) {
+            const uint32_t i = (next - base) * 256u + tid;
+            if (i < nbig) big_item<SPEC>(p, l, list[i], member % (unsigned)p.rep);
+        }
+        base += nchunk;
+    }
+    big_end(p, l);
+    const bool ok = big_grid_barrier(p.bar, members, ok_s);
+    if (ok && member == 0) {
+        if (tid < NLIST) {
+            p.big_count[tid * DSM_BIG_STRIDE] = 0u;
+            if (n_mine) atomicAdd(reinterpret_cast<unsigned long long *>(p.bar + DSM_BIGBAR_DRAWN), (unsigned long long)n_mine);
+        }
+    }
+    return ok;
+}
diff --git a/desman_amd/csrc/dsm_host.h b/desman_amd/csrc/dsm_host.h
--- a/desman_amd/csrc/dsm_host.h
+++ b/desman_amd/csrc/dsm_host.h
@@ -11,6 +11,11 @@
 #define DSM_BIG_NL 64
 #define DSM_BIG_STRIDE 16
 #define DSM_BIG_NT 3
+#define DSM_BIGBAR_CNT 0
+#define DSM_BIGBAR_GEN 16
+#define DSM_BIGBAR_ERR 32
+#define DSM_BIGBAR_DRAWN 48
+#define DSM_BIGBAR_WORDS 64
 #define DSM_U_CHUNK 8
 
 #define DSM_STATS_AGG 2
@@ -75,7 +80,11 @@
     int ntab_rep = 1;
     unsigned long long *big_list = nullptr;
     uint32_t *big_count = nullptr;
-    size_t big_cap = 0;
+    size_t big_cap = 0, big_seg = 0;
+    unsigned *big_bar = nullptr;
+    int big_helpers = -1, big_helpers_key = -1;
+    int big_inlaunch_mode = -1;
+    unsigned *h_big_err = nullptr;
     int stats_grid = 0;
     int stats_grid_key = -1;
     int item_stride = 1;
@@ -188,12 +197,13 @@
 int k_tau_rare_count(dsm_ctx *c, bool wait);
 int tau_rare_from_host(const double *gamma, int S, int G);
 int k_stats(dsm_ctx *c, uint32_t iter);
-int k_stats_stage1(dsm_ctx *c, uint32_t iter);
+int k_stats_stage1(dsm_ctx *c, uint32_t iter, bool big_in_consumer = false);
+int dirichlet_big_helpers(dsm_ctx *c);
 int k_stats_stage2(dsm_ctx *c, uint32_t iter);
 int k_binom_test(dsm_ctx *c, int kind, uint32_t n, const double *w, uint64_t seed, int nsamp, uint32_t *d_out, int spec);
 int k_esum_fold(dsm_ctx *c);
 int k_dirichlet(dsm_ctx *c, uint32_t iter, double *gamma_out, double *gamma_trace, double *eta_out, double *eta_trace,
-                double *prior_out, int fin_it, int fin_nblocks, const double *fin_prior, int do_s2 = 0);
+                double *prior_out, int fin_it, int fin_nblocks, const double *fin_prior, int do_s2 = 0, int big_helpers = -1);
 int k_prior(dsm_ctx *c, const double *gamma, const double *eta, double *prior_out);
 int k_prior_batch(dsm_ctx *c, const double *gamma, const double *eta, int n, double *prior_out);
 struct TauFinalRider { int nblocks, it; const double *prior, *gamma_src, *eta_src; };
diff --git a/desman_amd/csrc/kernels_gibbs.hip b/desman_amd/csrc/kernels_gibbs.hip
--- a/desman_amd/csrc/kernels_gibbs.hip
+++ b/desman_amd/csrc/kernels_gibbs.hip
@@ -5,6 +5,7 @@
 #include "dsm_device.h"
 #include "dsm_host.h"
 #include "dsm_stage2.h"
+#include "dsm_big.h"
 #include "log_table.h"
 
 __global__ __launch_bounds__(256) void convert_counts_kernel(const int64_t *__restrict__ in,
@@ -566,7 +567,8 @@
     Stage2Params s2;
 };
 
-__device__ __forceinline__ void dirichlet_body(const DirParams &q, const S2Plan &plan)
+template <bool BIG>
+__device__ __forceinline__ void dirichlet_body(const DirParams &q, const S2Plan &plan, const BigParams &big)
 {
     unsigned long long *__restrict__ sum_mu = q.sum_mu, *__restrict__ esum = q.esum;
     const int S = q.S, G = q.G;
@@ -578,12 +580,24 @@
     const int do_fin = q.do_fin, do_s2 = q.do_s2;
     const FinalParams &fin = q.fin;
     const Stage2Params &s2 = q.s2;
-    __shared__ __attribute__((aligned(16))) char smem_d[S2_SMEM_BYTES];
+    constexpr int SMEM_D = (BIG && DSM_BIG_INL_SMEM_BYTES > S2_SMEM_BYTES) ? DSM_BIG_INL_SMEM_BYTES : S2_SMEM_BYTES;
+    __shared__ __attribute__((aligned(16))) char smem_d[SMEM_D];
     if (do_fin && (int)blockIdx.x == S + 4) {
         double *red = reinterpret_cast<double *>(smem_d), *redp = red + 256;
         int *flag = reinterpret_cast<int *>(redp + 256);
         finalize_body(fin, red, redp, flag, threadIdx.x, 256);
         return;
+    }
+    if constexpr (BIG) {
+        if (big.bar) {
+            const uint32_t n_mine = threadIdx.x < DSM_BIG_NT * DSM_BIG_NL ? big.big_count[threadIdx.x * DSM_BIG_STRIDE] : 0u;
+            if (__syncthreads_or(n_mine != 0u)) {
+                const uint32_t member = blockIdx.x - ((do_fin && (int)blockIdx.x > S + 4) ? 1u : 0u), members = gridDim.x - (do_fin ? 1u : 0u);
+                const bool ok = do_s2 >= 3 ? big_inlaunch<3>(big, smem_d, n_mine, member, members) : big_inlaunch<2>(big, smem_d, n_mine, member, members);
+                if (!ok) return;
+            }
+            if ((int)blockIdx.x >= S + 4 + (do_fin ? 1 : 0)) return;
+        }
     }
     const int row = blockIdx.x;
     const bool is_gamma = row < S;
@@ -639,8 +653,8 @@
 #endif
 
 struct DirBatch { DirParams p[DSM_MAX_BATCH]; S2Plan plan; };
-__global__ __launch_bounds__(256) void dirichlet_kernel(DirParams q, S2Plan plan) { dirichlet_body(q, plan); }
-__global__ __launch_bounds__(256) void dirichlet_kernel_b(DirBatch b) { dirichlet_body(b.p[blockIdx.y], b.plan); }
+__global__ __launch_bounds__(256) void dirichlet_kernel(DirParams q, S2Plan plan, BigParams big) { dirichlet_body<true>(q, plan, big); }
+__global__ __launch_bounds__(256) void dirichlet_kernel_b(DirBatch b) { dirichlet_body<false>(b.p[blockIdx.y], b.plan, BigParams{}); }
 static_assert(sizeof(DirBatch) <= 4096, "kernarg segment");
 
 __global__ __launch_bounds__(256) void prior_kernel(const double *__restrict__ gamma, const double *__restrict__ eta,
@@ -1178,8 +1192,30 @@
     return p;
 }
 
+int dirichlet_big_helpers(dsm_ctx *c)
+{
+    const int key = ((c->S * 64 + c->G) * 2 + (c->tau_rng == DSM_RNG_MT19937 ? 1 : 0)) * 4 + (c->big_inlaunch_mode + 1);
+    if (c->big_helpers_key == key) return c->big_helpers;
+    c->big_helpers_key = key; c->big_helpers = -1;
+    if (c->big_inlaunch_mode == 0) return -1;
+    if (c->big_inlaunch_mode < 0 && (double)c->max_depth / (double)std::max(1, c->V) * 0.04 > DSM_LEAN_CAP) return -1;
+    int occ = 0;
+    hipDeviceProp_t prop;
+    if (hipOccupancyMaxActiveBlocksPerMultiprocessor(&occ, dirichlet_kernel, 256, 0) != hipSuccess ||
+        hipGetDeviceProperties(&prop, c->device) != hipSuccess) { (void)hipGetLastError(); return -1; }
+    const int n_xcd = prop.multiProcessorCount % 8 == 0 && prop.multiProcessorCount >= 64 ? 8 : 1;
+    const int cus = prop.multiProcessorCount - (c->tau_rng == DSM_RNG_MT19937 ? n_xcd : 0);
+    const int per_cu = std::min(2, occ - 1), rows = c->S + 4 + 1;
+    const long cap = (long)per_cu * cus;
+    if (per_cu < 1 || cap < rows) return -1;
+    long helpers = cap - rows;
+    if (const char *e = DSM_AB_ENV("DESMAN_HIP_BIG_HELPERS")) helpers = std::max(0L, std::min(helpers, atol(e)));
+    c->big_helpers = (int)helpers;
+    return c->big_helpers;
+}
+
 int k_dirichlet(dsm_ctx *c, uint32_t iter, double *gamma_out, double *gamma_trace, double *eta_out, double *eta_trace,
-                double *prior_out, int fin_it, int fin_nblocks, const double *fin_prior, int do_s2)
+                double *prior_out, int fin_it, int fin_nblocks, const double *fin_prior, int do_s2, int big_helpers)
 {
     KTimer tm(c, DSM_K_DIRICH);
     double lg, le;
@@ -1194,7 +1230,19 @@
     if (do_s2) {
         s2.ntab = c->ntab; s2.rep = c->ntab_rep; s2.ld = c->ntab_ld; s2.gamma = c->gamma; s2.sum_mu = c->sum_mu; s2.log_tab = c->log_tab;
         s2.S = c->S; s2.G = c->G; s2.k0 = k0; s2.k1 = k1; s2.iter = iter; s2.hmul = DSM_NTAB_HMUL; s2.swz = DSM_NTAB_SWZ;
-        s2.big_count = c->big_count;
+        s2.big_count = big_helpers >= 0 ? nullptr : c->big_count;
+    }
+    BigParams big = {};
+    if (big_helpers >= 0) {
+        if (!do_s2 || g_batch.K || c->shard_on || !c->big_bar) { dsm_set_error("k_dirichlet: deferred items in a launch without stage 2"); return DSM_ERR_STATE; }
+        big.cnt_vs = c->cnt_vs; big.tau = c->tau; big.gamma = c->gamma; big.eta = c->eta;
+        big.S = c->S; big.G = c->G; big.v_off = 0; big.V_tot = c->V;
+        big.k0 = k0; big.k1 = k1; big.iter = iter;
+        big.ntab = c->ntab; big.rep = c->ntab_rep; big.ld = c->ntab_ld; big.esum = c->esum; big.log_tab = c->log_tab;
+        big.big_list = c->big_list; big.big_count = c->big_count; big.big_seg = c->big_seg;
+        big.swz = DSM_NTAB_SWZ; big.hmul = DSM_NTAB_HMUL;
+        big.pat_x = stats_spec(c) == 4 ? c->pat_x : nullptr;
+        big.bar = c->big_bar;
     }
     DirParams q;
     q.sum_mu = c->sum_mu; q.esum = c->esum; q.S = c->S; q.G = c->G;
@@ -1204,7 +1252,7 @@
     q.do_fin = do_fin; q.fin = fin; q.do_s2 = do_s2 ? stats_draw_version(stats_spec(c)) : 0; q.s2 = s2;
     if (g_batch.K == 0) {
         const S2Plan plan = do_s2 ? make_stage2_plan(c->G) : S2Plan{};
-        hipLaunchKernelGGL(dirichlet_kernel, dim3(c->S + 4 + do_fin), dim3(256), 0, c->stream, q, plan);
+        hipLaunchKernelGGL(dirichlet_kernel, dim3(c->S + 4 + do_fin + std::max(0, big_helpers)), dim3(256), 0, c->stream, q, plan, big);
     } else {
         static thread_local DirBatch acc;
         acc.p[g_batch.k] = q;
diff --git a/desman_amd/csrc/kernels_stats.hip b/desman_amd/csrc/kernels_stats.hip
--- a/desman_amd/csrc/kernels_stats.hip
+++ b/desman_amd/csrc/kernels_stats.hip
@@ -1,3 +1,4 @@
+#include "dsm_big.h"
 #include "dsm_binom.h"
 #include "dsm_host.h"
 #include "log_table.h"
@@ -350,71 +351,16 @@
 template <int SPEC>
 __device__ __forceinline__ void stats_big_body(const StatsAggParams &p)
 {
-    __shared__ double2 ltab[DSM_LOG_TAB_N + DSM_EXP_TAB_N / 2];
-    __shared__ double rcp[DSM_RCP_TAB_N];
-    __shared__ double es[16];
-    __shared__ unsigned long long acc[16];
-    __shared__ uint32_t eacc[16 * 256];
-    const int tid = threadIdx.x, lane = tid & 63;
+    __shared__ __attribute__((aligned(16))) char smem_b[DSM_BIG_SMEM_BYTES];
+    const int tid = threadIdx.x;
     const uint32_t sub = blockIdx.x % (DSM_BIG_NT * DSM_BIG_NL), bi = blockIdx.x / (DSM_BIG_NT * DSM_BIG_NL), nb = gridDim.x / (DSM_BIG_NT * DSM_BIG_NL);
     const uint32_t nbig = p.big_count[sub * DSM_BIG_STRIDE];
     if (bi * 256u >= nbig) return;
     const unsigned long long *list = p.big_list + (size_t)sub * p.big_seg;
-    ltab[tid] = reinterpret_cast<const double2 *>(p.log_tab)[tid];
-    if (tid < DSM_EXP_TAB_N / 2) ltab[DSM_LOG_TAB_N + tid] = reinterpret_cast<const double2 *>(p.log_tab)[DSM_LOG_TAB_N + tid];
-    for (int k = tid; k < DSM_RCP_TAB_N; k += blockDim.x) rcp[k] = k ? 1.0 / (double)k : 0.0;
-    if (tid < 16) { es[tid] = p.eta[tid]; acc[tid] = 0ull; }
-#pragma unroll
-    for (int i = 0; i < 16; ++i) eacc[i * 256 + tid] = 0u;
-    __syncthreads();
-    const int S = p.S, G = p.G;
-    for (uint32_t i = bi * 256u + tid; i < nbig; i += nb * 256u) {
-        const unsigned long long item = list[i];
-        const uint32_t cell = (uint32_t)(item >> 2);
-        const int b = (int)(item & 3ull);
-        const int s = (int)(cell / (uint32_t)p.V_tot), v = (int)(cell - (uint32_t)s * (uint32_t)p.V_tot) - p.v_off;
-        const uint64_t t = p.tau[v];
-        uint32_t xb;
-        if (p.pat_x) { uint32_t *xw = p.pat_x + ((size_t)v * 4 + b) * S + s; xb = *xw; *xw = 0u; }
-        else xb = (uint32_t)p.cnt_vs[((size_t)v * S + s) * 4 + b];
-        uint32_t H[4] = {0, 0, 0, 0};
-        double Gam[4] = {0.0, 0.0, 0.0, 0.0};
-        for (int g = 0; g < G; ++g) {
-            const int a = (int)((t >> (2 * g)) & 3);
-            const double x = p.gamma[(size_t)s * G + g];
-#pragma unroll
-            for (int k = 0; k < 4; ++k) if (a == k) { H[k] |= 1u << g; Gam[k] = Gam[k] + x; }
-        }
-        double W[4];
-#pragma unroll
-        for (int a = 0; a < 4; ++a) W[a] = es[a * 4 + b] * Gam[a];
-        const double Wt = ((W[0] + W[1]) + W[2]) + W[3];
-        if (!(Wt > 0.0)) {
-#pragma unroll
-            for (int a = 0; a < 4; ++a) W[a] = Gam[a];
-        }
-        uint32_t n[4], cbase[4];
-        philox4x32_10(cell, 0u, p.iter, DSM_STREAM_STA1, p.k0, p.k1, cbase);
-        Xo128 rng = item_seed<SPEC>(cbase, (uint32_t)b, p.k0, p.k1);
-        bool defer = false;
-        mult4<true, SPEC>(rng, xb, W, n, rcp, ltab, defer);
-        uint32_t *erow = eacc + (b * 4) * 256 + tid;
-#pragma unroll
-        for (int a = 0; a < 4; ++a) {
-            erow[a * 256] += n[a];
-            if (n[a]) atomicAdd(p.ntab + (size_t)(blockIdx.x % (unsigned)p.rep) * (((size_t)1 << G) * (size_t)p.ld) + (size_t)((H[a] * p.hmul + ((uint32_t)s >> 4) * p.swz) & ((1u << G) - 1u)) * (size_t)p.ld + s, n[a]);
-        }
-    }
-    {
-        uint32_t e[16];
-#pragma unroll
-        for (int i = 0; i < 16; ++i) e[i] = eacc[i * 256 + tid];
-        const uint32_t tot = wave_transpose_reduce<16>(e);
-        const int idx = transpose_index<16>(lane);
-        if (lane < 16 && tot) atomicAdd(&acc[idx], (unsigned long long)tot);
-    }
-    __syncthreads();
-    if (tid < 16 && acc[tid]) atomicAdd(&p.esum[tid], acc[tid]);
+    const BigLds l = big_lds(smem_b);
+    big_begin(p, l);
+    for (uint32_t i = bi * 256u + tid; i < nbig; i += nb * 256u) big_item<SPEC>(p, l, list[i], blockIdx.x % (unsigned)p.rep);
+    big_end(p, l);
 }
 
 __global__ __launch_bounds__(256) void esum_fold_kernel(unsigned long long *__restrict__ esum)
@@ -567,6 +513,11 @@
         hipError_t e = hipMalloc((void **)&c->big_count, DSM_BIG_NT * DSM_BIG_NL * DSM_BIG_STRIDE * sizeof(uint32_t));
         if (e != hipSuccess) { dsm_set_error("hipMalloc failed: %s", hipGetErrorString(e)); return DSM_ERR_NOMEM; }
     }
+    if (!c->big_bar) {
+        hipError_t e = hipMalloc((void **)&c->big_bar, DSM_BIGBAR_WORDS * sizeof(unsigned));
+        if (e != hipSuccess) { dsm_set_error("hipMalloc failed: %s", hipGetErrorString(e)); return DSM_ERR_NOMEM; }
+        HIP_TRY(hipMemsetAsync(c->big_bar, 0, DSM_BIGBAR_WORDS * sizeof(unsigned), c->stream));
+    }
     hipError_t e = hipMalloc((void **)&c->big_list, need * sizeof(unsigned long long));
     if (e != hipSuccess) { dsm_set_error("hipMalloc(%zu B) failed: %s", need * 8, hipGetErrorString(e)); return DSM_ERR_NOMEM; }
     c->big_cap = need;
@@ -601,7 +552,7 @@
     return DSM_OK;
 }
 
-int k_stats_stage1(dsm_ctx *c, uint32_t iter)
+int k_stats_stage1(dsm_ctx *c, uint32_t iter, bool big_in_consumer)
 {
     int r = ensure_ntab(c);
     if (r != DSM_OK) return r;
@@ -643,6 +594,7 @@
     const size_t seg = (size_t)std::min<long>((long)V * S * 4, ((grid + DSM_BIG_NL - 1) / DSM_BIG_NL) * per_wg);
     r = ensure_big_list(c, seg);
     if (r != DSM_OK) return r;
+    c->big_seg = seg;
     StatsAggParams p;
     p.cnt_vs = c->cnt_vs; p.tau = c->tau; p.gamma = c->gamma; p.eta = c->eta;
     p.V = V; p.S = S; p.G = G; p.big_seg = seg;
@@ -711,6 +663,7 @@
         void *args[] = {(void *)&p};
         HIP_TRY(hipLaunchKernel(fn, dim3(grid), dim3(256), args, sh, c->stream));
     }
+    if (big_in_consumer) return DSM_OK;
     KTimer tm(c, DSM_K_STATSBIG);
     if (spec >= 3) hipLaunchKernelGGL(stats_big_kernel<3>, dim3(big_grid), dim3(256), 0, c->stream, p);
     else hipLaunchKernelGGL(stats_big_kernel<2>, dim3(big_grid), dim3(256), 0, c->stream, p);
diff --git a/include/desman_hip.h b/include/desman_hip.h
--- a/include/desman_hip.h
+++ b/include/desman_hip.h
@@ -66,6 +66,8 @@
 int dsm_ctx_stats_spec(dsm_ctx *ctx);
 int dsm_ctx_force_stats_spec(dsm_ctx *ctx, int spec);
 int dsm_ctx_debug_stage1(dsm_ctx *ctx, uint32_t iter, uint32_t *ntab, uint64_t *esum);
+int dsm_ctx_debug_deferred_drawn(dsm_ctx *ctx, uint64_t *drawn);
+int dsm_ctx_set_deferred_inlaunch(dsm_ctx *ctx, int mode);
 int dsm_ctx_debug_binom(dsm_ctx *ctx, int kind, uint32_t n, const double *w4, uint64_t seed, int nsamp,
                         uint32_t *out, int spec);
 
```
